# Neos-codes/microbeast

Measured on AMD Instinct MI355X. Metric: env frames/sec (whole node) on 16x16 microRTS, higher is better.
Workload: dtype bf16

## Files before the change

### microbeast_amd/csrc/env/microrts_sim.cpp

```cpp
#include "microrts_sim.h"
#include "../include/microrts_rules.h"
#include <algorithm>
#include <cstring>
#include <cstdlib>
#include <stdexcept>

namespace mb {

#define MB_SPEC(t)                                                                          \
  {(int16_t)mbr::spec_hp(t), (int16_t)mbr::spec_cost(t), (int16_t)mbr::spec_damage(t),      \
   (int16_t)mbr::spec_range(t), (int16_t)mbr::spec_move_t(t), (int16_t)mbr::spec_attack_t(t), \
   (int16_t)mbr::spec_produce_t(t)}
const UnitSpec kSpec[8] = {MB_SPEC(0), MB_SPEC(1), MB_SPEC(2), MB_SPEC(3),
                           MB_SPEC(4), MB_SPEC(5), MB_SPEC(6), MB_SPEC(7)};
#undef MB_SPEC
static constexpr int kHarvestT = mbr::kHarvestT, kReturnT = mbr::kReturnT;
static constexpr int kDX[4] = {0, 1, 0, -1};
static constexpr int kDY[4] = {-1, 0, 1, 0};

enum { R_WIN = 0, R_RES = 1, R_WORKER = 2, R_BUILD = 3, R_ATTACK = 4, R_COMBAT = 5 };

static inline void setbit(uint32_t* w, int j) { w[j >> 5] |= 1u << (j & 31); }
static inline bool getbit(const uint32_t* w, int j) { return (w[j >> 5] >> (j & 31)) & 1u; }

MicroRTSSim::MicroRTSSim(int size, int max_steps, int bot, uint64_t seed, const float* rw)
    : s_(size), max_steps_(max_steps), bot_(bot) {
  if (size < 1 || size > 32) throw std::invalid_argument("MicroRTSSim: map size must be 1..32");
  static const float def[kNumRewards] = {10.f, 1.f, 1.f, 0.2f, 1.f, 4.f};
  for (int i = 0; i < kNumRewards; ++i) rw_[i] = rw ? rw[i] : def[i];
  uint64_t z = seed + 0x9E3779B97F4A7C15ull;
  z = (z ^ (z >> 30)) * 0xBF58476D1CE4E5B9ull;
  z = (z ^ (z >> 27)) * 0x94D049BB133111EBull;
  rng_ = (z ^ (z >> 31)) | 1ull;
  grid_.assign(s_ * s_, -1);
  act_buf_.assign((size_t)s_ * s_ * kActComps, 0);
  mask_.assign(s_ * s_ * kMaskWords, 0u);
  mask_p1_.assign(s_ * s_ * kMaskWords, 0u);
  opp_actions_.assign(s_ * s_ * kActComps, 0);
  reset();
}

uint32_t MicroRTSSim::rand_u32() {
  rng_ ^= rng_ << 13; rng_ ^= rng_ >> 7; rng_ ^= rng_ << 17;
  return (uint32_t)(rng_ >> 16);
}
float MicroRTSSim::rand_unit() { return (rand_u32() & 0xFFFFFF) * (1.f / 16777216.f); }

int MicroRTSSim::add_unit(int type, int owner, int x, int y, int res) {
  Unit u{};
  u.x = x; u.y = y; u.type = type; u.owner = owner;
  u.hp = kSpec[type].hp; u.res = res; u.busy = 0; u.act = A_NOOP; u.alive = 1;
  int uid = -1;
  for (size_t i = 0; i < units_.size(); ++i)
    if (!units_[i].alive) { uid = (int)i; break; }
  if (uid < 0) { uid = (int)units_.size(); units_.push_back(u); }
  else units_[uid] = u;
  grid_[cell(x, y)] = (int16_t)uid;
  if (owner >= 0) ++cnt_[owner][type];
  last_add_ = uid;
  return uid;
}

void MicroRTSSim::kill(int uid) {
  Unit& u = units_[uid];
  if (!u.alive) return;
  grid_[cell(u.x, u.y)] = -1;
  u.alive = 0;
  if (u.owner >= 0) --cnt_[u.owner][u.type];
}

void MicroRTSSim::reset() {
  units_.clear();
  units_.reserve((size_t)s_ * s_ + 4);
  std::memset(cnt_, 0, sizeof(cnt_));
  std::fill(grid_.begin(), grid_.end(), (int16_t)-1);
  tick_ = 0;
  resources_[0] = resources_[1] = 5;
  const int o = s_ >= 8 ? 1 : 0;
  const int b = s_ >= 8 ? 2 : 1;
  for (int p = 0; p < 2; ++p) {
    auto X = [&](int x) { return p == 0 ? x : s_ - 1 - x; };
    auto Y = [&](int y) { return p == 0 ? y : s_ - 1 - y; };
    add_unit(RESOURCE, -1, X(0), Y(0), s_ >= 8 ? 20 : 10);
    if (s_ >= 8) add_unit(RESOURCE, -1, X(0), Y(1), 20);
    add_unit(BASE, p, X(b), Y(b));
    add_unit(WORKER, p, X(o), Y(b == 1 ? 0 : o), 0);
    if (s_ >= 12) add_unit(WORKER, p, X(b + 1), Y(b), 0);
  }
  if (validate_) compute_mask(0, mask_);
  if (external_opp_ && validate_) compute_mask(1, mask_p1_);
}

void MicroRTSSim::unit_mask(const Unit& u, int player, uint32_t* w) const {
  w[0] = w[1] = w[2] = 0;
  if (!u.alive || u.owner != player || u.busy > 0 || u.type == RESOURCE) return;
  const UnitSpec& sp = kSpec[u.type];
  setbit(w, kNvecOff[0] + A_NOOP);
  bool any_move = false, any_harv = false, any_ret = false, any_prod = false, any_att = false;
  const bool mobile = u.type >= WORKER;
  for (int d = 0; d < 4; ++d) {
    int nx = u.x + kDX[d], ny = u.y + kDY[d];
    if (!in_bounds(nx, ny)) continue;
    int g = grid_[cell(nx, ny)];
    if (g < 0) {
      if (mobile) { setbit(w, kNvecOff[1] + d); any_move = true; }
      bool can_prod = false;
      if (u.type == BASE && resources_[player] >= kSpec[WORKER].cost) can_prod = true;
      if (u.type == BARRACKS && resources_[player] >= kSpec[LIGHT].cost) can_prod = true;
      if (u.type == WORKER && resources_[player] >= kSpec[BARRACKS].cost) can_prod = true;
      if (can_prod) { setbit(w, kNvecOff[4] + d); any_prod = true; }
    } else {
      const Unit& t = units_[g];
      if (u.type == WORKER && t.type == RESOURCE && u.res == 0 && t.res > 0) {
        setbit(w, kNvecOff[2] + d); any_harv = true;
      }
      if (u.type == WORKER && t.type == BASE && t.owner == player && u.res > 0) {
        setbit(w, kNvecOff[3] + d); any_ret = true;
      }
    }
  }
  if (any_prod) {
    const int r = resources_[player];
    if (u.type == BASE) setbit(w, kNvecOff[5] + (WORKER - 1));
    if (u.type == BARRACKS) {
      if (r >= kSpec[LIGHT].cost) setbit(w, kNvecOff[5] + (LIGHT - 1));
      if (r >= kSpec[HEAVY].cost) setbit(w, kNvecOff[5] + (HEAVY - 1));
      if (r >= kSpec[RANGED].cost) setbit(w, kNvecOff[5] + (RANGED - 1));
    }
    if (u.type == WORKER) {
      if (r >= kSpec[BASE].cost) setbit(w, kNvecOff[5] + (BASE - 1));
      if (r >= kSpec[BARRACKS].cost) setbit(w, kNvecOff[5] + (BARRACKS - 1));
    }
  }
  if (sp.damage > 0) {
    const int R = sp.range, Rs = std::min(R, 3);
    for (int ay = -Rs; ay <= Rs; ++ay)
      for (int ax = -Rs; ax <= Rs; ++ax) {
        if (ax * ax + ay * ay > R * R || (ax == 0 && ay == 0)) continue;
        int tx = u.x + ax, ty = u.y + ay;
        if (!in_bounds(tx, ty)) continue;
        int g = grid_[cell(tx, ty)];
        if (g >= 0 && units_[g].owner == 1 - player) {
          setbit(w, kNvecOff[6] + (ay + 3) * 7 + (ax + 3)); any_att = true;
        }
      }
  }
  if (any_move) setbit(w, kNvecOff[0] + A_MOVE);
  if (any_harv) setbit(w, kNvecOff[0] + A_HARVEST);
  if (any_ret) setbit(w, kNvecOff[0] + A_RETURN);
  if (any_prod) setbit(w, kNvecOff[0] + A_PRODUCE);
  if (any_att) setbit(w, kNvecOff[0] + A_ATTACK);
}

static void mirror_mask_bits(const uint32_t* in, uint32_t* out) {
  out[0] = out[1] = out[2] = 0;
  for (int j = 0; j < kMaskBits; ++j) {
    if (!getbit(in, j)) continue;
    int k = j;
    if (j >= kNvecOff[1] && j < kNvecOff[5]) {
      int g = (j - kNvecOff[1]) / 4, d = (j - kNvecOff[1]) % 4;
      k = kNvecOff[1] + g * 4 + (d + 2) % 4;
    } else if (j >= kNvecOff[6]) {
      int a = j - kNvecOff[6];
      k = kNvecOff[6] + (6 - a / 7) * 7 + (6 - a % 7);
    }
    setbit(out, k);
  }
}

void MicroRTSSim::map_xy(int player, int x, int y, int* ox, int* oy) const {
  if (player == 0) { *ox = x; *oy = y; }
  else { *ox = s_ - 1 - x; *oy = s_ - 1 - y; }
}

void MicroRTSSim::compute_mask(int player, std::vector<uint32_t>& out) const {
  std::fill(out.begin(), out.end(), 0u);
  for (const Unit& u : units_) {
    if (!u.alive || u.owner != player || u.busy > 0) continue;
    uint32_t w[3];
    unit_mask(u, player, w);
    int px, py;
    map_xy(player, u.x, u.y, &px, &py);
    uint32_t* dst = &out[(size_t)cell(px, py) * kMaskWords];
    if (player == 0) { dst[0] = w[0]; dst[1] = w[1]; dst[2] = w[2]; }
    else mirror_mask_bits(w, dst);
  }
}

bool MicroRTSSim::exec(int uid, const uint8_t* a, float* rw) {
  Unit& u = units_[uid];
  if (!u.alive || u.busy > 0) return false;
  const int player = u.owner;
  const UnitSpec& sp = kSpec[u.type];
  switch (a[0]) {
    case A_NOOP: return true;
    case A_MOVE: {
      if (u.type < WORKER) return false;
      int d = a[1] & 3, nx = u.x + kDX[d], ny = u.y + kDY[d];
      if (!empty(nx, ny)) return false;
      grid_[cell(u.x, u.y)] = -1;
      u.x = nx; u.y = ny;
      grid_[cell(nx, ny)] = (int16_t)uid;
      u.busy = sp.move_t; u.act = A_MOVE;
      return true;
    }
    case A_HARVEST: {
      int d = a[2] & 3, nx = u.x + kDX[d], ny = u.y + kDY[d];
      if (u.type != WORKER || u.res > 0 || !in_bounds(nx, ny)) return false;
      int g = grid_[cell(nx, ny)];
      if (g < 0 || units_[g].type != RESOURCE || units_[g].res <= 0) return false;
      units_[g].res -= 1; u.res = 1;
      if (units_[g].res <= 0) kill(g);
      u.busy = kHarvestT; u.act = A_HARVEST;
      if (rw) rw[R_RES] += 1.f;
      return true;
    }
    case A_RETURN: {
      int d = a[3] & 3, nx = u.x + kDX[d], ny = u.y + kDY[d];
      if (u.type != WORKER || u.res <= 0 || !in_bounds(nx, ny)) return false;
      int g = grid_[cell(nx, ny)];
      if (g < 0 || units_[g].type != BASE || units_[g].owner != player) return false;
      resources_[player] += u.res; u.res = 0;
      u.busy = kReturnT; u.act = A_RETURN;
      if (rw) rw[R_RES] += 1.f;
      return true;
    }
    case A_PRODUCE: {
      int d = a[4] & 3, nx = u.x + kDX[d], ny = u.y + kDY[d];
      int t = (int)a[5] + 1;
      if (t < 1 || t > 7 || !empty(nx, ny)) return false;
      bool ok = (u.type == BASE && t == WORKER) ||
                (u.type == BARRACKS && (t == LIGHT || t == HEAVY || t == RANGED)) ||
                (u.type == WORKER && (t == BASE || t == BARRACKS));
      if (!ok || resources_[player] < kSpec[t].cost) return false;
      resources_[player] -= kSpec[t].cost;
      int nu = add_unit(t, player, nx, ny);
      Unit& uu = units_[uid];
      units_[nu].busy = kSpec[t].produce_t;
      units_[nu].act = A_PRODUCE;
      uu.busy = kSpec[t].produce_t; uu.act = A_PRODUCE;
      if (rw) {
        if (t == WORKER) rw[R_WORKER] += 1.f;
        else if (t == BASE || t == BARRACKS) rw[R_BUILD] += 1.f;
        else rw[R_COMBAT] += 1.f;
      }
      return true;
    }
    case A_ATTACK: {
      if (sp.damage <= 0) return false;
      int ax = (int)(a[6] % 7) - 3, ay = (int)(a[6] / 7) - 3;
      if (ax * ax + ay * ay > sp.range * sp.range) return false;
      int tx = u.x + ax, ty = u.y + ay;
      if (!in_bounds(tx, ty)) return false;
      int g = grid_[cell(tx, ty)];
      if (g < 0 || units_[g].owner != 1 - player) return false;
      units_[g].hp -= sp.damage;
      if (units_[g].hp <= 0) kill(g);
      u.busy = sp.attack_t; u.act = A_ATTACK;
      if (rw) rw[R_ATTACK] += 1.f;
      return true;
    }
  }
  return false;
}

int MicroRTSSim::nearest(int uid, int owner_filter, int type_filter, int* dist) const {
  const Unit& u = units_[uid];
  int best = -1, bd = 1 << 30;
  for (size_t i = 0; i < units_.size(); ++i) {
    const Unit& t = units_[i];
    if (!t.alive || (int)i == uid) continue;
    if (owner_filter != -2 && t.owner != owner_filter) continue;
    if (type_filter > 0 && t.type != type_filter) continue;
    int d = std::abs(t.x - u.x) + std::abs(t.y - u.y);
    if (d < bd) { bd = d; best = (int)i; }
  }
  if (dist) *dist = bd;
  return best;
}

int MicroRTSSim::dir_toward(const Unit& u, int tx, int ty) const {
  int best = -1, bd = 1 << 30;
  const int d0 = std::abs(tx - u.x) + std::abs(ty - u.y);
  for (int d = 0; d < 4; ++d) {
    int nx = u.x + kDX[d], ny = u.y + kDY[d];
    if (!empty(nx, ny)) continue;
    int dd = std::abs(tx - nx) + std::abs(ty - ny);
    if (dd < bd) { bd = dd; best = d; }
  }
  if (best < 0 || bd < d0) return best;
  const int S = s_ * s_;
  int16_t dist[32 * 32];
  int16_t q[32 * 32];
  if (S > 32 * 32) return best;
  std::fill(dist, dist + S, (int16_t)-1);
  int qh = 0, qt = 0;
  const int tc = cell(tx, ty);
  dist[tc] = 0;
  q[qt++] = (int16_t)tc;
  while (qh < qt) {
    const int c = q[qh++], cx = c % s_, cy = c / s_;
    for (int d = 0; d < 4; ++d) {
      const int nx = cx + kDX[d], ny = cy + kDY[d];
      if (!in_bounds(nx, ny)) continue;
      const int nc = cell(nx, ny);
      if (dist[nc] >= 0) continue;
      if (nx == u.x && ny == u.y) {
        for (int k = 0; k < 4; ++k)
          if (u.x + kDX[k] == cx && u.y + kDY[k] == cy) return empty(cx, cy) ? k : best;
      }
      if (grid_[nc] >= 0) continue;
      dist[nc] = (int16_t)(dist[c] + 1);
      q[qt++] = (int16_t)nc;
    }
  }
  return best;
}

static constexpr int kCoacWorkers = 8, kCoacHarvesters = 1;
static constexpr int kLightWorkers = 3;
static constexpr bool kChaseBaseFirst = true;
static constexpr int kChaseBaseSlack = 3;
static constexpr int kRBToward = 8;
static constexpr bool kHuntNoBase = true;
static constexpr bool kHuntAll = false;

void MicroRTSSim::bot_unit(int uid, int player, float* rwo, int n_workers, int n_barracks,
                           int widx) {
  Unit& u = units_[uid];
  uint8_t a[7] = {0, 0, 0, 0, 0, 0, 0};
  const int enemy = 1 - player;
  auto try_attack = [&]() -> bool {
    const UnitSpec& sp = kSpec[u.type];
    if (sp.damage <= 0) return false;
    int best = -1, bkey = 1 << 30;
    const int Rs = std::min<int>(sp.range, 3);
    for (int ay = -Rs; ay <= Rs; ++ay)
      for (int ax = -Rs; ax <= Rs; ++ax) {
        if (ax * ax + ay * ay > sp.range * sp.range || (ax == 0 && ay == 0)) continue;
        int tx = u.x + ax, ty = u.y + ay;
        if (!in_bounds(tx, ty)) continue;
        int g = grid_[cell(tx, ty)];
        if (g >= 0 && units_[g].owner == enemy) {
          const Unit& t = units_[g];
          const int key = (kSpec[t.type].damage > 0 ? 0 : 64) + t.hp;
          if (key < bkey) { bkey = key; best = (ay + 3) * 7 + (ax + 3); }
        }
      }
    if (best < 0) return false;
    a[0] = A_ATTACK; a[6] = (uint8_t)best;
    return exec(uid, a, rwo);
  };
  auto move_to = [&](int tx, int ty) -> bool {
    int d = dir_toward(u, tx, ty);
    if (d < 0) return false;
    a[0] = A_MOVE; a[1] = (uint8_t)d;
    return exec(uid, a, rwo);
  };
  auto produce = [&](int type) -> bool {
    for (int k = 0; k < 4; ++k) {
      int d = (int)((rand_u32() + k) & 3);
      if (!empty(u.x + kDX[d], u.y + kDY[d])) continue;
      a[0] = A_PRODUCE; a[4] = (uint8_t)d; a[5] = (uint8_t)(type - 1);
      return exec(uid, a, rwo);
    }
    return false;
  };
  auto harvest_cycle = [&]() -> bool {
    if (u.res > 0) {
      int dist, b = nearest(uid, player, BASE, &dist);
      if (b < 0) return false;
      if (dist == 1) {
        for (int d = 0; d < 4; ++d)
          if (u.x + kDX[d] == units_[b].x && u.y + kDY[d] == units_[b].y) {
            a[0] = A_RETURN; a[3] = (uint8_t)d; return exec(uid, a, rwo);
          }
      }
      return move_to(units_[b].x, units_[b].y);
    }
    int dist, r = nearest(uid, -1, RESOURCE, &dist);
    if (r < 0) return false;
    if (dist == 1) {
      for (int d = 0; d < 4; ++d)
        if (u.x + kDX[d] == units_[r].x && u.y + kDY[d] == units_[r].y) {
          a[0] = A_HARVEST; a[2] = (uint8_t)d; return exec(uid, a, rwo);
        }
    }
    return move_to(units_[r].x, units_[r].y);
  };
  auto chase = [&]() -> bool {
    int e = -1, dist = 1 << 30, b = -1, db = 1 << 30;
    for (size_t i = 0; i < units_.size(); ++i) {
      const Unit& t = units_[i];
      if (!t.alive || t.owner != enemy) continue;
      const int d = std::abs(t.x - u.x) + std::abs(t.y - u.y);
      if (d < dist) { dist = d; e = (int)i; }
      if (t.type == BASE && d < db) { db = d; b = (int)i; }
    }
    if (e < 0) return false;
    if (kChaseBaseFirst && b >= 0 && db <= dist + kChaseBaseSlack) e = b;
    return move_to(units_[e].x, units_[e].y);
  };

  switch (bot_) {
    case BOT_PASSIVE: return;
    case BOT_RANDOM_BIASED: {
      if (kHuntNoBase && u.type >= WORKER && count_units(enemy, BASE) == 0) {
        if (try_attack()) return;
        if (chase()) return;
      }
      uint32_t w[3];
      unit_mask(u, player, w);
      struct Cand { uint8_t t, p0, p1; };
      Cand cand[4 + 4 + 4 + 4 * 7 + 49 + 1];
      int wt[sizeof(cand) / sizeof(cand[0])], n = 0, tot = 0;
      auto add = [&](uint8_t t, uint8_t p0, uint8_t p1, int weight) {
        cand[n] = {t, p0, p1};
        wt[n++] = weight;
        tot += weight;
      };
      add(A_NOOP, 0, 0, 1);
      int ed = -1, ex = 0, ey = 0;
      if (kRBToward > 1 && u.type >= WORKER) {
        const int e = nearest(uid, 1 - player, -1, &ed);
        if (e >= 0) { ex = units_[e].x; ey = units_[e].y; } else { ed = -1; }
      }
      for (int d = 0; d < 4; ++d) {
        if (getbit(w, kNvecOff[1] + d)) {
          const int nd = std::abs(ex - (u.x + kDX[d])) + std::abs(ey - (u.y + kDY[d]));
          add(A_MOVE, (uint8_t)d, 0, ed >= 0 && nd < ed ? kRBToward : 1);
        }
        if (getbit(w, kNvecOff[2] + d)) add(A_HARVEST, (uint8_t)d, 0, 5);
        if (getbit(w, kNvecOff[3] + d)) add(A_RETURN, (uint8_t)d, 0, 5);
        if (getbit(w, kNvecOff[4] + d))
          for (int k = 0; k < 7; ++k)
            if (getbit(w, kNvecOff[5] + k)) add(A_PRODUCE, (uint8_t)d, (uint8_t)k, 1);
      }
      if (getbit(w, kNvecOff[0] + A_ATTACK))
        for (int j = 0; j < 49; ++j)
          if (getbit(w, kNvecOff[6] + j)) add(A_ATTACK, (uint8_t)j, 0, 5);
      int r = (int)(rand_u32() % (uint32_t)tot), k = 0;
      while (r >= wt[k]) r -= wt[k++];
      const Cand c = cand[k];
      if (c.t == A_NOOP) return;
      a[0] = c.t;
      switch (c.t) {
        case A_MOVE: a[1] = c.p0; break;
        case A_HARVEST: a[2] = c.p0; break;
        case A_RETURN: a[3] = c.p0; break;
        case A_PRODUCE: a[4] = c.p0; a[5] = c.p1; break;
        case A_ATTACK: a[6] = c.p0; break;
        default: break;
      }
      exec(uid, a, rwo);
      return;
    }
    case BOT_RANDOM: {
      uint32_t w[3];
      unit_mask(u, player, w);
      int at = A_NOOP;
      {
        int c[6], n = 0;
        for (int k = 0; k < 6; ++k) if (getbit(w, k)) c[n++] = k;
        at = n ? c[rand_u32() % n] : A_NOOP;
      }
      a[0] = (uint8_t)at;
      int comps[2] = {0, 0}, nc = 0;
      switch (at) {
        case A_MOVE: comps[nc++] = 1; break;
        case A_HARVEST: comps[nc++] = 2; break;
        case A_RETURN: comps[nc++] = 3; break;
        case A_PRODUCE: comps[nc++] = 4; comps[nc++] = 5; break;
        case A_ATTACK: comps[nc++] = 6; break;
        default: break;
      }
      for (int k = 0; k < nc; ++k) {
        const int comp = comps[k];
        int cand[49], n = 0;
        for (int j = 0; j < kNvec[comp]; ++j)
          if (getbit(w, kNvecOff[comp] + j)) cand[n++] = j;
        a[comp] = n ? (uint8_t)cand[rand_u32() % n] : 0;
      }
      if (at != A_NOOP) exec(uid, a, rwo);
      return;
    }
    case BOT_WORKER_RUSH: {
      if (u.type == BASE) { produce(WORKER); return; }
      if (u.type == WORKER) {
        if (try_attack()) return;
        if (widx == 0 && !(kHuntAll && count_units(enemy, BASE) == 0) && harvest_cycle()) return;
        chase();
      }
      return;
    }
    case BOT_LIGHT_RUSH: {
      if (u.type == BASE) { if (n_workers < kLightWorkers) produce(WORKER); return; }
      if (u.type == BARRACKS) { produce(LIGHT); return; }
      if (u.type == WORKER) {
        if (try_attack()) return;
        if (n_barracks == 0 && resources_[player] >= kSpec[BARRACKS].cost && widx == 0) {
          if (produce(BARRACKS)) return;
        }
        if (widx < kLightWorkers - 1 && harvest_cycle()) return;
        chase();
        return;
      }
      if (try_attack()) return;
      chase();
      return;
    }
    case BOT_COAC:
    default: {
      if (u.type == BASE) { if (n_workers < kCoacWorkers) produce(WORKER); return; }
      if (u.type == BARRACKS) {
        const int r = resources_[player];
        int t = (r >= kSpec[HEAVY].cost && rand_unit() < 0.3f) ? HEAVY
              : (rand_unit() < 0.5f ? RANGED : LIGHT);
        produce(t);
        return;
      }
      if (u.type == WORKER) {
        if (try_attack()) return;
        if (n_barracks == 0 && n_workers >= kCoacWorkers / 2 &&
            resources_[player] >= kSpec[BARRACKS].cost && widx == 1) {
          if (produce(BARRACKS)) return;
        }
        if (widx < kCoacHarvesters && !(kHuntAll && count_units(enemy, BASE) == 0) &&
            harvest_cycle())
          return;
        chase();
        return;
      }
      if (try_attack()) return;
      chase();
      return;
    }
  }
}

void MicroRTSSim::bot_act(int player, float* rwo) {
  const int n_workers = cnt_[player][WORKER], n_barracks = cnt_[player][BARRACKS];
  const int n = (int)units_.size();
  uint16_t cand[32 * 32 + 4], cw[32 * 32 + 4], added[32 * 32 + 4];
  int nc = 0, w = 0, na = 0;
  for (int i = 0; i < n; ++i) {
    const Unit& u = units_[i];
    const int own = (u.alive != 0) & (u.owner == player);
    cand[nc] = (uint16_t)i;
    cw[nc] = (uint16_t)w;
    nc += own & (u.busy == 0);
    w += own & (u.type == WORKER);
  }
  for (int q = 0; q < nc; ++q) {
    const int i = cand[q];
    int widx = cw[q];
    for (int t = 0; t < na; ++t) widx += added[t] < i;
    last_add_ = -1;
    bot_unit(i, player, rwo, n_workers, n_barracks, widx);
    const int k = last_add_;
    if (k > i && k < n && units_[k].type == WORKER && units_[k].owner == player)
      added[na++] = (uint16_t)k;
  }
}

void MicroRTSSim::set_opponent_actions(const uint8_t* a) {
  std::memcpy(opp_actions_.data(), a, opp_actions_.size());
}

float MicroRTSSim::step(const uint8_t* actions, bool* done, float* raw) {
  float rw[kNumRewards] = {0, 0, 0, 0, 0, 0};
  const int nc = s_ * s_;
  uint32_t idle[32 * 32 + 4];
  int n_idle = 0;
  for (size_t i = 0; i < units_.size(); ++i) {
    const Unit& u = units_[i];
    idle[n_idle] = ((uint32_t)cell(u.x, u.y) << 16) | (uint32_t)i;
    n_idle += (u.alive != 0) & (u.owner == 0) & (u.busy == 0);
  }
  for (int q = 1; q < n_idle; ++q) {
    const uint32_t key = idle[q];
    int j = q;
    for (; j > 0 && idle[j - 1] > key; --j) idle[j] = idle[j - 1];
    idle[j] = key;
  }
  for (int q = 0; q < n_idle; ++q) {
    const uint32_t key = idle[q];
    const int c = (int)(key >> 16), g = (int)(key & 0xFFFFu);
    uint8_t tmp[kActComps];
    const uint8_t* a = actions + (size_t)c * kActComps;
    if (p16_) {
      mbr::unpack_env_action(p16_[c], tmp);
      a = tmp;
    }
    if (!validate_) {
      if (a[0] < 6) exec(g, a, rw);
      continue;
    }
    const uint32_t* m = &mask_[(size_t)c * kMaskWords];
    if (a[0] >= 6 || !getbit(m, a[0])) continue;
    int comp = 0;
    switch (a[0]) {
      case A_MOVE: comp = 1; break; case A_HARVEST: comp = 2; break;
      case A_RETURN: comp = 3; break; case A_PRODUCE: comp = 4; break;
      case A_ATTACK: comp = 6; break; default: comp = 0;
    }
    if (comp && (a[comp] >= kNvec[comp] || !getbit(m, kNvecOff[comp] + a[comp]))) continue;
    if (a[0] == A_PRODUCE && (a[5] >= 7 || !getbit(m, kNvecOff[5] + a[5]))) continue;
    exec(g, a, rw);
  }
  if (external_opp_) {
    for (int c = 0; c < nc; ++c) {
      int rx, ry;
      map_xy(1, c % s_, c / s_, &rx, &ry);
      const int g = grid_[cell(rx, ry)];
      if (g < 0) continue;
      const Unit& u = units_[g];
      if (u.owner != 1 || u.busy > 0) continue;
      uint8_t otmp[kActComps];
      const uint8_t* ap = &opp_actions_[(size_t)c * kActComps];
      if (opp16_) {
        mbr::unpack_env_action(opp16_[c], otmp);
        ap = otmp;
      }
      if (ap[0] >= 6) continue;
      if (validate_ && !getbit(&mask_p1_[(size_t)c * kMaskWords], ap[0])) continue;
      uint8_t a[7];
      for (int k = 0; k < 7; ++k) a[k] = ap[k];
      for (int k = 1; k <= 4; ++k) a[k] = (uint8_t)((ap[k] + 2) & 3);
      a[6] = (uint8_t)((6 - ap[6] / 7) * 7 + (6 - ap[6] % 7));
      exec(g, a, nullptr);
    }
  } else {
    bot_act(1, nullptr);
  }
  ++tick_;
  int alive[2] = {0, 0};
  for (int t = 0; t < 8; ++t) {
    alive[0] += cnt_[0][t];
    alive[1] += cnt_[1][t];
  }
  bool d = false;
  if (alive[1] == 0 || alive[0] == 0) {
    d = true;
    last_winner_ = alive[1] == 0 ? (alive[0] == 0 ? -1 : 0) : 1;
    rw[R_WIN] = last_winner_ == 0 ? 1.f : (last_winner_ == 1 ? -1.f : 0.f);
  } else if (tick_ >= max_steps_) {
    d = true;
    last_winner_ = -1;
  }
  int rows_n = 0, rows_idle = 0;
  if (!d && rows_out_) {
    uint32_t spill;
    for (Unit& u : units_) {
      const int16_t b = u.busy, nb = (int16_t)(b - (u.alive && b > 0));
      u.act = (b > 0 && nb == 0 && u.alive) ? (int8_t)A_NOOP : u.act;
      u.busy = nb;
      const int live = u.alive != 0;
      rows_idle += live & (u.owner == 0) & (u.act == A_NOOP);
      *(rows_n < nc ? rows_out_ + rows_n : &spill) = row_entry(u, 0);
      rows_n += live;
    }
  } else if (!d) {
    for (Unit& u : units_) {
      const int16_t b = u.busy, nb = (int16_t)(b - (u.alive && b > 0));
      u.act = (b > 0 && nb == 0 && u.alive) ? (int8_t)A_NOOP : u.act;
      u.busy = nb;
    }
  }
  float r = 0.f;
  for (int i = 0; i < kNumRewards; ++i) r += rw_[i] * rw[i];
  if (raw) for (int i = 0; i < kNumRewards; ++i) raw[i] = rw[i];
  *done = d;
  if (d) {
    reset();
    if (rows_out_) rows_n = write_obs_code_list(rows_out_, &rows_idle);
  }
  rows_n_ = rows_n;
  rows_idle_ = rows_idle;
  if (!d) {
    if (validate_) compute_mask(0, mask_);
    if (external_opp_ && validate_) compute_mask(1, mask_p1_);
  }
  return r;
}

float MicroRTSSim::step_packed_list(const uint16_t* env_actions, bool* done, uint32_t* entries,
                                    int* n, int* idle_own) {
  rows_out_ = entries;
  const float r = step_packed(env_actions, done);
  rows_out_ = nullptr;
  *n = rows_n_;
  if (idle_own) *idle_own += rows_idle_;
  return r;
}

float MicroRTSSim::step_packed2_list(const uint16_t* env_actions, const uint16_t* opp_actions,
                                     bool* done, uint32_t* entries, int* n, int* idle_own) {
  rows_out_ = entries;
  const float r = step_packed2(env_actions, opp_actions, done);
  rows_out_ = nullptr;
  *n = rows_n_;
  if (idle_own) *idle_own += rows_idle_;
  return r;
}

float MicroRTSSim::step_packed(const uint16_t* env_actions, bool* done) {
  p16_ = env_actions;
  const float r = step(nullptr, done, nullptr);
  p16_ = nullptr;
  return r;
}

float MicroRTSSim::step_packed2(const uint16_t* env_actions, const uint16_t* opp_actions,
                                bool* done) {
  opp16_ = opp_actions;
  const float r = step_packed(env_actions, done);
  opp16_ = nullptr;
  return r;
}

void MicroRTSSim::write_obs_codes_as(int player, uint16_t* out) const {
  const int nc = s_ * s_;
  std::memset(out, 0, (size_t)nc * sizeof(uint16_t));
  for (const Unit& u : units_) {
    if (!u.alive) continue;
    int px, py;
    map_xy(player, u.x, u.y, &px, &py);
    const int own = u.owner < 0 ? 0 : (u.owner == player ? 1 : 2);
    out[cell(px, py)] = mbr::cell_code(std::min<int>(std::max<int>(u.hp, 0), 4),
                                       std::min<int>(std::max<int>(u.res, 0), 4), own, u.type,
                                       u.act);
  }
}

int MicroRTSSim::write_obs_code_list(uint32_t* entries, int* idle_own, int player) const {
  const int S = s_ * s_;
  uint32_t spill;
  int n = 0, idle = 0;
  for (const Unit& u : units_) {
    const int live = u.alive != 0;
    idle += live & (u.owner == player) & (u.act == A_NOOP);
    *(n < S ? entries + n : &spill) = row_entry(u, player);
    n += live;
  }
  if (idle_own) *idle_own += idle;
  return n;
}

static inline uint32_t unit_bits(const Unit* u, int player) {
  if (!u) return (1u << 0) | (1u << 5) | (1u << 10) | (1u << 13) | (1u << 21);
  uint32_t b = 0;
  b |= 1u << (0 + std::min<int>(std::max<int>(u->hp, 0), 4));
  b |= 1u << (5 + std::min<int>(std::max<int>(u->res, 0), 4));
  int own = u->owner < 0 ? 0 : (u->owner == player ? 1 : 2);
  b |= 1u << (10 + own);
  b |= 1u << (13 + u->type);
  b |= 1u << (21 + u->act);
  return b;
}

void MicroRTSSim::write_obs(uint32_t* out) const {
  const int nc = s_ * s_;
  for (int c = 0; c < nc; ++c) {
    int g = grid_[c];
    out[c] = unit_bits(g >= 0 ? &units_[g] : nullptr, 0);
  }
}

void MicroRTSSim::write_obs_p1(uint32_t* out) const {
  const int nc = s_ * s_;
  for (int c = 0; c < nc; ++c) {
    int rx, ry;
    map_xy(1, c % s_, c / s_, &rx, &ry);
    int g = grid_[cell(rx, ry)];
    out[c] = unit_bits(g >= 0 ? &units_[g] : nullptr, 1);
  }
}

void MicroRTSSim::write_mask(uint32_t* out) const {
  std::memcpy(out, mask_.data(), mask_.size() * sizeof(uint32_t));
}
void MicroRTSSim::write_mask_p1(uint32_t* out) const {
  std::memcpy(out, mask_p1_.data(), mask_p1_.size() * sizeof(uint32_t));
}

void MicroRTSSim::write_obs_dense(float* out) const {
  const int nc = s_ * s_;
  for (int c = 0; c < nc; ++c) {
    int g = grid_[c];
    uint32_t b = unit_bits(g >= 0 ? &units_[g] : nullptr, 0);
    for (int p = 0; p < kPlanes; ++p) out[(size_t)c * kPlanes + p] = (float)((b >> p) & 1u);
  }
}

void MicroRTSSim::write_mask_dense(uint8_t* out) const {
  const int nc = s_ * s_;
  for (int c = 0; c < nc; ++c)
    for (int j = 0; j < kMaskBits; ++j)
      out[(size_t)c * kMaskBits + j] = getbit(&mask_[(size_t)c * kMaskWords], j) ? 1 : 0;
}

}
```

### microbeast_amd/csrc/env/microrts_sim.h

```cpp
#pragma once
#include <cstdint>
#include <vector>
#include <string>

namespace mb {

constexpr int kPlanes = 27;
constexpr int kMaskBits = 78;
constexpr int kMaskWords = 3;
constexpr int kActComps = 7;
constexpr int kNvec[kActComps] = {6, 4, 4, 4, 4, 7, 49};
constexpr int kNvecOff[kActComps + 1] = {0, 6, 10, 14, 18, 22, 29, 78};
constexpr int kNumRewards = 6;

enum UnitType : int8_t { NONE = 0, RESOURCE = 1, BASE = 2, BARRACKS = 3, WORKER = 4,
                         LIGHT = 5, HEAVY = 6, RANGED = 7 };
enum ActType : int8_t { A_NOOP = 0, A_MOVE = 1, A_HARVEST = 2, A_RETURN = 3,
                        A_PRODUCE = 4, A_ATTACK = 5 };
enum Bot : int8_t { BOT_COAC = 0, BOT_RANDOM_BIASED = 1, BOT_LIGHT_RUSH = 2,
                    BOT_WORKER_RUSH = 3, BOT_PASSIVE = 4, BOT_RANDOM = 5 };

struct Unit {
  int16_t x, y;
  int8_t type;
  int8_t owner;
  int16_t hp;
  int16_t res;
  int16_t busy;
  int8_t act;
  int8_t alive;
};

struct SimStats {
  float ep_return = 0.f;
  int32_t ep_step = 0;
};

class MicroRTSSim {
 public:
  MicroRTSSim(int size, int max_steps, int bot, uint64_t seed,
              const float* reward_weight );
  void reset();
  float step(const uint8_t* actions, bool* done, float* raw_rewards );
  void write_obs(uint32_t* out) const;
  void write_mask(uint32_t* out) const;
  void write_obs_dense(float* out) const;
  void write_mask_dense(uint8_t* out) const;
  int size() const { return s_; }
  void prefetch() const {
    const char* u = (const char*)units_.data();
    for (size_t o = 0; o < units_.size() * sizeof(Unit); o += 64) __builtin_prefetch(u + o);
    const char* g = (const char*)grid_.data();
    for (size_t o = 0; o < grid_.size() * sizeof(int16_t); o += 64) __builtin_prefetch(g + o);
  }
  int bot() const { return bot_; }
  void set_bot(int b) { bot_ = b; }
  int winner() const { return last_winner_; }
  int ticks() const { return tick_; }
  void set_external_opponent(bool on) {
    external_opp_ = on;
    if (on && validate_) compute_mask(1, mask_p1_);
  }
  void write_obs_p1(uint32_t* out) const;
  void write_mask_p1(uint32_t* out) const;
  void set_opponent_actions(const uint8_t* actions_p1);
  void set_validate(bool on) {
    validate_ = on;
    if (on) {
      compute_mask(0, mask_);
      if (external_opp_) compute_mask(1, mask_p1_);
    }
  }
  float step_packed(const uint16_t* env_actions, bool* done);
  float step_packed_list(const uint16_t* env_actions, bool* done, uint32_t* entries, int* n,
                         int* idle_own);
  float step_packed2_list(const uint16_t* env_actions, const uint16_t* opp_actions, bool* done,
                          uint32_t* entries, int* n, int* idle_own);
  float step_packed2(const uint16_t* env_actions, const uint16_t* opp_actions, bool* done);
  void write_obs_codes(uint16_t* out) const { write_obs_codes_as(0, out); }
  int write_obs_code_list(uint32_t* entries, int* idle_own = nullptr, int player = 0) const;
  void write_obs_codes_as(int player, uint16_t* out) const;
  bool external_opponent() const { return external_opp_; }
  int resources(int player) const { return resources_[player]; }
  int count_units(int owner, int type) const {
    if (owner < 0 || owner > 1) {
      int n = 0;
      for (const Unit& u : units_) n += u.alive && u.owner == owner && (type < 0 || u.type == type);
      return n;
    }
    if (type >= 0) return cnt_[owner][type];
    int n = 0;
    for (int t = 0; t < 8; ++t) n += cnt_[owner][t];
    return n;
  }

 private:
  int s_, max_steps_, bot_;
  uint64_t rng_;
  float rw_[kNumRewards];
  int tick_ = 0;
  int resources_[2] = {0, 0};
  int last_winner_ = -1;
  bool external_opp_ = false;
  bool validate_ = true;
  std::vector<uint8_t> act_buf_;
  std::vector<Unit> units_;
  std::vector<int16_t> grid_;
  std::vector<uint32_t> mask_;
  std::vector<uint32_t> mask_p1_;
  std::vector<uint8_t> opp_actions_;
  int cnt_[2][8] = {};
  const uint16_t* p16_ = nullptr;
  const uint16_t* opp16_ = nullptr;
  uint32_t* rows_out_ = nullptr;
  int rows_n_ = 0, rows_idle_ = 0;
  int last_add_ = -1;

  uint32_t rand_u32();
  float rand_unit();
  int cell(int x, int y) const { return y * s_ + x; }
  uint32_t row_entry(const Unit& u, int player) const {
    const int px = player ? s_ - 1 - u.x : u.x, py = player ? s_ - 1 - u.y : u.y;
    const int own = u.owner < 0 ? 0 : (u.owner == player ? 1 : 2);
    const int hp = u.hp < 0 ? 0 : (u.hp > 4 ? 4 : u.hp);
    const int res = u.res < 0 ? 0 : (u.res > 4 ? 4 : u.res);
    return (uint32_t)cell(px, py) |
           ((uint32_t)(hp | (res << 3) | (own << 6) | (u.type << 8) | (u.act << 11)) << 16);
  }
  bool in_bounds(int x, int y) const { return x >= 0 && y >= 0 && x < s_ && y < s_; }
  bool empty(int x, int y) const { return in_bounds(x, y) && grid_[cell(x, y)] < 0; }
  int add_unit(int type, int owner, int x, int y, int res = 0);
  void kill(int uid);
  void compute_mask(int player, std::vector<uint32_t>& out) const;
  void unit_mask(const Unit& u, int player, uint32_t* w) const;
  bool exec(int uid, const uint8_t* a, float* rw);
  void bot_act(int player, float* rw_opp);
  void bot_unit(int uid, int player, float* rw_opp, int n_workers, int n_barracks, int widx);
  int nearest(int uid, int owner_filter, int type_filter, int* dist) const;
  int dir_toward(const Unit& u, int tx, int ty) const;
  void map_xy(int player, int x, int y, int* ox, int* oy) const;
};

struct UnitSpec { int16_t hp, cost, damage, range, move_t, attack_t, produce_t; };
extern const UnitSpec kSpec[8];

}
```

### microbeast_amd/csrc/runtime/engine.cpp

```cpp
#include "engine.h"


#include <chrono>
#include <cstdlib>

#include <pthread.h>
#include <sched.h>
#include <cstring>
#include <stdexcept>
#include <string>

#include "../include/mbk_api.h"

namespace mb {

#define ENG_CHECK(expr)                                                              \
  do {                                                                               \
    hipError_t _e = (expr);                                                          \
    if (_e != hipSuccess) {                                                          \
      fail(std::string(#expr) + " failed: " + hipGetErrorString(_e));                \
      return false;                                                                  \
    }                                                                                \
  } while (0)

#define CTOR_CHECK(expr)                                                             \
  do {                                                                               \
    hipError_t _e = (expr);                                                          \
    if (_e != hipSuccess)                                                            \
      throw std::runtime_error(std::string(#expr) + " failed: " + hipGetErrorString(_e)); \
  } while (0)

GpuEngine::GpuEngine(const EngineConfig& cfg, const EngineBuffers& buf) : cfg_(cfg), buf_(buf) {
  if (cfg_.n_groups < 1 || cfg_.envs_per_group < 1 || cfg_.unroll < 1)
    throw std::runtime_error("GpuEngine: bad config");
  if (cfg_.n_slots < cfg_.n_groups + 1)
    throw std::runtime_error("GpuEngine: need n_slots >= n_groups + 1");
  S_ = cfg_.size * cfg_.size;
  const size_t E = cfg_.envs_per_group, T1 = cfg_.unroll + 1;
  slot_stride_obs_ = T1 * E * S_ * 4;
  slot_stride_mask_ = T1 * E * S_ * 4 * kMaskWords;
  slot_stride_act_ = T1 * E * S_ * kActComps;
  slot_stride_scalar_ = T1 * E;
  const int total = cfg_.n_groups * cfg_.envs_per_group;
  env_.reset(new VecEnv(cfg_.size, total, cfg_.max_steps, cfg_.seed, cfg_.bots,
                        cfg_.reward_weight.empty() ? nullptr : cfg_.reward_weight.data(),
                        cfg_.env_index_base));
  CTOR_CHECK(hipSetDevice(cfg_.device));
  if (cfg_.n_lanes < 1 || (int)buf_.lanes.size() != cfg_.n_lanes)
    throw std::runtime_error("GpuEngine: need one LaneIO per lane");
  int prio_least = 0, prio_greatest = 0;
  CTOR_CHECK(hipDeviceGetStreamPriorityRange(&prio_least, &prio_greatest));
  lanes_.resize(cfg_.n_lanes);
  for (int l = 0; l < cfg_.n_lanes; ++l) {
    Lane& L = lanes_[l];
    L.io = buf_.lanes[l];
    if (!L.io.in_codes || !L.io.in_res || !L.io.out_act16)
      throw std::runtime_error("GpuEngine: in_codes / in_res / out_act16 buffers required");
    CTOR_CHECK(hipStreamCreateWithPriority(&L.stream, hipStreamNonBlocking, prio_greatest));
  }
  CTOR_CHECK(hipHostMalloc((void**)&h_codes_, (size_t)total * S_ * 2, hipHostMallocDefault));
  CTOR_CHECK(hipHostMalloc((void**)&h_res_, (size_t)total * 4, hipHostMallocDefault));
  CTOR_CHECK(hipHostMalloc((void**)&h_act16_, (size_t)total * S_ * 2, hipHostMallocDefault));
  CTOR_CHECK(hipHostMalloc((void**)&h_reward_, (size_t)total * 4, hipHostMallocDefault));
  CTOR_CHECK(hipHostMalloc((void**)&h_done_, (size_t)total, hipHostMallocDefault));
  std::memset(h_reward_, 0, (size_t)total * 4);
  std::memset(h_done_, 0, (size_t)total);
  if (buf_.ep_return || buf_.ep_step) {
    CTOR_CHECK(hipHostMalloc((void**)&h_ep_return_, (size_t)total * 4, hipHostMallocDefault));
    CTOR_CHECK(hipHostMalloc((void**)&h_ep_step_, (size_t)total * 4, hipHostMallocDefault));
    std::memset(h_ep_return_, 0, (size_t)total * 4);
    std::memset(h_ep_step_, 0, (size_t)total * 4);
  }
  if (cfg_.selfplay_groups < 0 || cfg_.selfplay_groups > cfg_.n_groups)
    throw std::runtime_error("GpuEngine: bad selfplay_groups");
  const int sp0 = cfg_.n_groups - cfg_.selfplay_groups;
  if (cfg_.selfplay_groups > 0) {
    for (const Lane& L : lanes_)
      if (!L.io.in_codes_p1 || !L.io.in_res_p1 || !L.io.out_act16_p1)
        throw std::runtime_error(
            "GpuEngine: self-play needs in_codes_p1 / in_res_p1 / out_act16_p1");
    CTOR_CHECK(hipHostMalloc((void**)&h_codes_p1_, (size_t)total * S_ * 2, hipHostMallocDefault));
    CTOR_CHECK(hipHostMalloc((void**)&h_res_p1_, (size_t)total * 4, hipHostMallocDefault));
    CTOR_CHECK(hipHostMalloc((void**)&h_act16_p1_, (size_t)total * S_ * 2, hipHostMallocDefault));
    std::memset(h_act16_p1_, 0, (size_t)total * S_ * 2);
    env_->set_external_opponent(sp0 * cfg_.envs_per_group, total, true);
  }
  if (cfg_.preroll > 1) {
    env_->reset_codes(nullptr, nullptr);
    preroll_steps_ = env_->preroll(cfg_.preroll, cfg_.seed, std::max(1, cfg_.n_threads));
    env_->set_validate(false);
    env_->write_codes(h_codes_, h_res_);
  } else {
    env_->set_validate(false);
    env_->reset_codes(h_codes_, h_res_);
  }
  if (cfg_.selfplay_groups > 0) env_->reset_codes_p1(h_codes_p1_, h_res_p1_);
  {
    const char* st = std::getenv("MBK_STEP_TIMING");
    step_timing_ = st && st[0] == '1';
  }
  for (int g = 0; g < cfg_.n_groups; ++g) {
    groups_.emplace_back(new Group());
    CTOR_CHECK(hipEventCreateWithFlags(&groups_[g]->ev, hipEventDisableTiming));
    if (step_timing_)
      for (auto& e : groups_[g]->tev) CTOR_CHECK(hipEventCreate(&e));
    groups_[g]->selfplay = g >= sp0;
    groups_[g]->lane = g % cfg_.n_lanes;
    groups_[g]->phase.store(READY);
  }
  full_ev_.resize(cfg_.n_slots);
  release_ev_.resize(cfg_.n_slots);
  release_pending_.assign(cfg_.n_slots, 0);
  slot_version_.assign(cfg_.n_slots, 0);
  for (int s = 0; s < cfg_.n_slots; ++s) {
    CTOR_CHECK(hipEventCreateWithFlags(&full_ev_[s], hipEventDisableTiming));
    CTOR_CHECK(hipEventCreateWithFlags(&release_ev_[s], hipEventDisableTiming));
    free_slots_.push_back(s);
  }
  for (PubChan& c : pub_) {
    CTOR_CHECK(hipEventCreateWithFlags(&c.ready, hipEventDisableTiming));
    c.pending.assign(cfg_.n_lanes, false);
    c.dst.assign(cfg_.n_lanes, 0);
    c.consumed.assign(cfg_.n_lanes, nullptr);
    for (auto& ev : c.consumed) CTOR_CHECK(hipEventCreateWithFlags(&ev, hipEventDisableTiming));
  }
  chunk_ = std::max(1, std::min(16, cfg_.envs_per_group / std::max(1, 2 * cfg_.n_threads)));
}

GpuEngine::~GpuEngine() {
  stop();
  for (Lane& L : lanes_)
    if (L.stream) hipStreamSynchronize(L.stream);
  for (auto& g : groups_) {
    if (g->ev) hipEventDestroy(g->ev);
    for (auto e : g->tev)
      if (e) hipEventDestroy(e);
  }
  for (auto e : full_ev_) hipEventDestroy(e);
  for (auto e : release_ev_) hipEventDestroy(e);
  for (PubChan& c : pub_) {
    if (c.ready) hipEventDestroy(c.ready);
    for (auto ev : c.consumed)
      if (ev) hipEventDestroy(ev);
    if (c.staging) hipFree(c.staging);
  }
  if (h_codes_p1_) hipHostFree(h_codes_p1_);
  if (h_res_p1_) hipHostFree(h_res_p1_);
  if (h_act16_p1_) hipHostFree(h_act16_p1_);
  if (h_codes_) hipHostFree(h_codes_);
  if (h_res_) hipHostFree(h_res_);
  if (h_act16_) hipHostFree(h_act16_);
  if (h_reward_) hipHostFree(h_reward_);
  if (h_ep_return_) hipHostFree(h_ep_return_);
  if (h_ep_step_) hipHostFree(h_ep_step_);
  if (h_done_) hipHostFree(h_done_);
  if (h_code_list_) hipHostFree(h_code_list_);
  if (h_act_list_) hipHostFree(h_act_list_);
  if (h_code_list_p1_) hipHostFree(h_code_list_p1_);
  if (h_act_list_p1_) hipHostFree(h_act_list_p1_);
  for (Lane& L : lanes_) {
    if (L.opp_scratch) hipFree(L.opp_scratch);
    if (L.stream) hipStreamDestroy(L.stream);
  }
}

void GpuEngine::fail(const std::string& msg) {
  {
    std::lock_guard<std::mutex> g(err_m_);
    if (err_.empty()) err_ = msg;
  }
  failed_.store(true);
  running_.store(false);
  work_cv_.notify_all();
  full_cv_.notify_all();
}

std::string GpuEngine::error() const {
  std::lock_guard<std::mutex> g(err_m_);
  return err_;
}

void GpuEngine::start(const std::vector<LaneGraphs>& graphs) {
  if (running_.load()) return;
  if ((int)graphs.size() != cfg_.n_lanes)
    throw std::runtime_error("GpuEngine::start: need one LaneGraphs per lane");
  for (int l = 0; l < cfg_.n_lanes; ++l) {
    const LaneGraphs& g = graphs[l];
    if (!g.policy) throw std::runtime_error("GpuEngine::start: missing policy graph");
    if (cfg_.selfplay_groups > 0 && !g.opp)
      throw std::runtime_error("GpuEngine::start: self-play groups need the opponent graph");
    Lane& L = lanes_[l];
    L.graph = (hipGraphExec_t)g.policy;
    L.opp_graph = (hipGraphExec_t)g.opp;
    L.pack_graph[0] = (hipGraphExec_t)g.pack;
    L.pack_graph[1] = (hipGraphExec_t)g.opp_pack;
  }
  started_ = true;
  running_.store(true);
  for (int w = 0; w < cfg_.n_threads; ++w) workers_.emplace_back(&GpuEngine::worker_loop, this, w);
  driver_ = std::thread(&GpuEngine::driver_loop, this);
}

void GpuEngine::alloc_rows() {
  if (h_code_list_) return;
  const size_t total = (size_t)cfg_.n_groups * cfg_.envs_per_group;
  list_stride_ = (S_ + 1 + 3) & ~3;
  const size_t bytes = total * list_stride_ * 4;
  if (hipHostMalloc((void**)&h_code_list_, bytes, hipHostMallocDefault) != hipSuccess ||
      hipHostMalloc((void**)&h_act_list_, bytes, hipHostMallocDefault) != hipSuccess)
    throw std::runtime_error("GpuEngine: hipHostMalloc of the sparse rows failed");
  std::memset(h_act_list_, 0, bytes);
  env_->write_code_lists(h_code_list_, list_stride_);
  if (cfg_.selfplay_groups > 0) {
    if (hipHostMalloc((void**)&h_code_list_p1_, bytes, hipHostMallocDefault) != hipSuccess ||
        hipHostMalloc((void**)&h_act_list_p1_, bytes, hipHostMallocDefault) != hipSuccess)
      throw std::runtime_error("GpuEngine: hipHostMalloc of the opponent rows failed");
    std::memset(h_act_list_p1_, 0, bytes);
    std::memset(h_code_list_p1_, 0, bytes);
    env_->write_code_lists(h_code_list_p1_, list_stride_, 1);
  }
}

void GpuEngine::set_greedy(bool on) {
  if (started_ || running_.load()) throw std::runtime_error("set_greedy: engine already started");
  greedy_ = on;
}

void GpuEngine::set_sparse_io(bool on) {
  if (running_.load()) throw std::runtime_error("set_sparse_io: engine running");
  if (!on) { sparse_ = false; return; }
  if (act_mode()) return;
  if (buf_.ep_return || buf_.ep_step)
    throw std::runtime_error("set_sparse_io: not with the reference buffer keys");
  alloc_rows();
  sparse_ = true;
}

void GpuEngine::set_act_models(const std::vector<MbkActModel>& models,
                               const std::vector<MbkActModel>& opp_models) {
  if (running_.load()) throw std::runtime_error("set_act_models: engine running");
  if (!models.empty() && (int)models.size() != cfg_.n_lanes)
    throw std::runtime_error("set_act_models: need one model per lane");
  if (!models.empty() && (buf_.ep_return || buf_.ep_step || buf_.last_action0 || buf_.logits))
    throw std::runtime_error("set_act_models: not with reference buffer keys");
  const bool sp_needed = !models.empty() && cfg_.selfplay_groups > 0;
  if (sp_needed && (int)opp_models.size() != cfg_.n_lanes)
    throw std::runtime_error("set_act_models: self-play needs one opponent block per lane");
  if (!sp_needed && !opp_models.empty())
    throw std::runtime_error("set_act_models: opponent blocks without self-play groups");
  for (const std::vector<MbkActModel>* v : {&models, &opp_models})
    for (const MbkActModel& m : *v)
      if (m.E != cfg_.envs_per_group || m.H != cfg_.size || m.W != cfg_.size)
        throw std::runtime_error("set_act_models: model block shape mismatch");
  act_models_ = models;
  opp_act_models_ = opp_models;
  sparse_ = !models.empty();
  if (sparse_) alloc_rows();
  if (sp_needed) {
    const size_t E = cfg_.envs_per_group, sc = E * S_ * (4 + 12 + 8) + 2 * E * 4 + 256;
    for (Lane& L : lanes_)
      if (!L.opp_scratch && hipMalloc((void**)&L.opp_scratch, sc) != hipSuccess)
        throw std::runtime_error("set_act_models: hipMalloc of the opponent scratch failed");
  }
}

void GpuEngine::stop() {
  running_.store(false);
  work_cv_.notify_all();
  full_cv_.notify_all();
  if (driver_.joinable()) driver_.join();
  for (auto& t : workers_) if (t.joinable()) t.join();
  workers_.clear();
  for (Lane& L : lanes_)
    if (L.stream) hipStreamSynchronize(L.stream);
}

void GpuEngine::dispatch_env(int g) {
  Group& G = *groups_[g];
  const auto now = std::chrono::steady_clock::now();
  gpu_phase_ns_.fetch_add(
      std::chrono::duration_cast<std::chrono::nanoseconds>(now - G.t_phase).count(),
      std::memory_order_relaxed);
  G.t_phase = now;
  if (G.timed) {
    float ms[3] = {0.f, 0.f, 0.f};
    bool ok = true;
    for (int i = 0; i < 3; ++i)
      ok = ok && hipEventElapsedTime(&ms[i], G.tev[i], G.tev[i + 1]) == hipSuccess;
    if (ok) {
      step_h2d_ns_.fetch_add((int64_t)(ms[0] * 1e6), std::memory_order_relaxed);
      step_graph_ns_.fetch_add((int64_t)(ms[1] * 1e6), std::memory_order_relaxed);
      step_out_ns_.fetch_add((int64_t)(ms[2] * 1e6), std::memory_order_relaxed);
      timed_steps_.fetch_add(1, std::memory_order_relaxed);
    }
    G.timed = false;
  }
  G.idle.store(0, std::memory_order_relaxed);
  G.phase.store(ENV_BUSY, std::memory_order_release);
  G.remaining.store(cfg_.envs_per_group, std::memory_order_release);
  G.next_env.store(0, std::memory_order_release);
  {
    std::lock_guard<std::mutex> l(work_m_);
    work_epoch_.fetch_add(1);
  }
  work_cv_.notify_all();
}

void GpuEngine::worker_loop(int wid) {
  const int E = cfg_.envs_per_group, NG = cfg_.n_groups;
  while (running_.load(std::memory_order_relaxed)) {
    const uint64_t epoch = work_epoch_.load();
    bool did = false;
    for (int k = 0; k < NG; ++k) {
      const int g = (wid + k) % NG;
      Group& G = *groups_[g];
      if (G.phase.load(std::memory_order_acquire) != ENV_BUSY) continue;
      for (;;) {
        int e = G.next_env.fetch_add(chunk_);
        if (e >= E) break;
        int e1 = std::min(e + chunk_, E);
        const int a0 = g * E;
        auto t0 = std::chrono::steady_clock::now();
        try {
          if (inject_fault_.exchange(0) != 0)
            throw std::runtime_error("injected env-worker fault (--fault_inject_every)");
          if (sparse_ && G.selfplay)
            G.idle.fetch_add(env_->step_range_lists_sp(a0 + e, a0 + e1, h_act_list_,
                                                       h_act_list_p1_, h_code_list_,
                                                       h_code_list_p1_, list_stride_, h_reward_,
                                                       h_done_, &log_, G.opp_version),
                             std::memory_order_relaxed);
          else if (sparse_)
            G.idle.fetch_add(env_->step_range_lists(a0 + e, a0 + e1, h_act_list_, h_code_list_,
                                                    list_stride_, h_reward_, h_done_, &log_),
                             std::memory_order_relaxed);
          else if (G.selfplay)
            env_->step_range_codes_sp(a0 + e, a0 + e1, h_act16_, h_act16_p1_, h_codes_, h_res_,
                                      h_codes_p1_, h_res_p1_, h_reward_, h_done_, &log_,
                                      G.opp_version, h_ep_return_, h_ep_step_);
          else
            env_->step_range_codes(a0 + e, a0 + e1, h_act16_, h_codes_, h_res_, h_reward_,
                                   h_done_, &log_, h_ep_return_, h_ep_step_);
        } catch (const std::exception& ex) {
          fail("env worker " + std::to_string(wid) + ": " + ex.what());
          return;
        }
        env_ns_.fetch_add(std::chrono::duration_cast<std::chrono::nanoseconds>(
                              std::chrono::steady_clock::now() - t0).count(),
                          std::memory_order_relaxed);
        frames_.fetch_add(e1 - e, std::memory_order_relaxed);
        did = true;
        if (G.remaining.fetch_sub(e1 - e) == e1 - e) {
          G.t_ready_ns.store(std::chrono::duration_cast<std::chrono::nanoseconds>(
                                 std::chrono::steady_clock::now().time_since_epoch()).count(),
                             std::memory_order_relaxed);
          G.phase.store(READY, std::memory_order_release);
        }
      }
    }
    if (!did) {
      std::unique_lock<std::mutex> l(work_m_);
      work_cv_.wait_for(l, std::chrono::milliseconds(2),
                        [&] { return work_epoch_.load() != epoch || !running_.load(); });
    }
  }
}

bool GpuEngine::enqueue_gpu(int g) {
  const auto t_enq = std::chrono::steady_clock::now();
  struct Timer {
    std::atomic<int64_t>& acc;
    std::chrono::steady_clock::time_point t0;
    ~Timer() {
      acc.fetch_add(std::chrono::duration_cast<std::chrono::nanoseconds>(
                        std::chrono::steady_clock::now() - t0).count(),
                    std::memory_order_relaxed);
    }
  } timer{enqueue_ns_, t_enq};
  Group& G = *groups_[g];
  Lane& L = lanes_[G.lane];
  hipStream_t st = L.stream;
  const LaneIO& io = L.io;
  const size_t E = cfg_.envs_per_group, T = cfg_.unroll;
  {
    std::lock_guard<std::mutex> l(pub_m_);
    const int ln = G.lane;
    for (int c = 0; c < 2; ++c) {
      PubChan& P = pub_[c];
      if (!P.pending[ln]) continue;
      if (hipEventQuery(P.ready) == hipErrorNotReady) continue;
      ENG_CHECK(hipStreamWaitEvent(st, P.ready, 0));
      ENG_CHECK(hipMemcpyAsync((void*)P.dst[ln], P.staging, P.n, hipMemcpyDeviceToDevice,
                               st));
      ENG_CHECK(hipEventRecord(P.consumed[ln], st));
      if (L.pack_graph[c]) ENG_CHECK(hipGraphLaunch(L.pack_graph[c], st));
      P.pending[ln] = false;
      if (c == 1) L.opp_version = P.version;
      else if (P.version >= 0) L.policy_version = P.version;
      bool all = true;
      for (bool pl : P.pending) all = all && !pl;
      if (all) {
        if (c == 0) publishes_.fetch_add(1);
        else {
          opp_version_pub_.store(P.version);
          opp_publishes_.fetch_add(1);
        }
      }
    }
  }
  if (G.t == 0) {
    auto waiting = [&] {
      for (int w : slot_wait_q_) if (w == g) return true;
      return false;
    };
    if (!slot_wait_q_.empty() && slot_wait_q_.front() != g) {
      if (!waiting()) slot_wait_q_.push_back(g);
      return false;
    }
    int slot = -1;
    bool pending = false;
    {
      std::lock_guard<std::mutex> l(slot_m_);
      for (auto it = free_slots_.begin(); it != free_slots_.end(); ++it) {
        const int s = *it;
        if (release_pending_[s]) {
          const hipError_t q = hipEventQuery(release_ev_[s]);
          if (q == hipErrorNotReady) continue;
          if (q == hipSuccess) release_pending_[s] = 0;
        }
        slot = s;
        pending = release_pending_[s] != 0;
        free_slots_.erase(it);
        break;
      }
    }
    if (slot < 0) {
      if (!waiting()) slot_wait_q_.push_back(g);
      return false;
    }
    if (!slot_wait_q_.empty() && slot_wait_q_.front() == g) slot_wait_q_.pop_front();
    if (pending) ENG_CHECK(hipStreamWaitEvent(st, release_ev_[slot], 0));
    G.cur = slot;
    slot_version_[slot] = L.policy_version;
  }
  const size_t e0 = (size_t)g * E;
  G.timed = step_timing_;
  const size_t t = G.t;
  auto obs_at = [&](int slot, size_t i) {
    return (char*)buf_.obs + slot * slot_stride_obs_ + i * E * S_ * 4;
  };
  auto mask_at = [&](int slot, size_t i) {
    return (char*)buf_.mask + slot * slot_stride_mask_ + i * E * S_ * 4 * kMaskWords;
  };
  auto act_at = [&](int slot, size_t i) {
    return (char*)buf_.action + slot * slot_stride_act_ + i * E * S_ * kActComps;
  };
  auto f32_at = [&](uintptr_t base, int slot, size_t i) {
    return (char*)base + (slot * slot_stride_scalar_ + i * E) * 4;
  };
  auto u8_at = [&](uintptr_t base, int slot, size_t i) {
    return (char*)base + (slot * slot_stride_scalar_ + i * E);
  };
  const bool close_prev = (t == 0 && G.prev >= 0);
  const int rs = t > 0 ? G.cur : G.prev;
  const size_t ri = t > 0 ? t - 1 : T - 1;
  if (act_mode()) {
    const MbkActModel& M = act_models_[G.lane];
    if (G.timed) ENG_CHECK(hipEventRecord(G.tev[0], st));
    if (G.timed) ENG_CHECK(hipEventRecord(G.tev[1], st));
    MbkActStep a{};
    a.code_list = h_code_list_ + e0 * list_stride_;
    a.act_list = h_act_list_ + e0 * list_stride_;
    a.list_stride = list_stride_;
    a.obs = (uint32_t*)obs_at(G.cur, t);
    a.mask = (uint32_t*)mask_at(G.cur, t);
    if (close_prev) {
      a.obs2 = (uint32_t*)obs_at(G.prev, T);
      a.mask2 = (uint32_t*)mask_at(G.prev, T);
    }
    a.action = (uint8_t*)act_at(G.cur, t);
    if (buf_.abits) {
      const size_t sw = (size_t)(S_ + 31) / 32;
      auto ab_at = [&](int slot, size_t i) {
        return (uint32_t*)buf_.abits + (slot * slot_stride_scalar_ + i * E) * sw;
      };
      a.abits = ab_at(G.cur, t);
      if (close_prev) a.abits2 = ab_at(G.prev, T);
    }
    a.logp = (float*)f32_at(buf_.logp, G.cur, t);
    a.value = (float*)f32_at(buf_.value, G.cur, t);
    if (!G.first) {
      a.reward_src = h_reward_ + e0;
      a.done_src = h_done_ + e0;
      a.reward_dst = (float*)f32_at(buf_.reward, rs, ri);
      a.done_dst = (uint8_t*)u8_at(buf_.done, rs, ri);
    }
    a.step = L.act_step++;
    a.greedy = greedy_ ? 1 : 0;
    act_active_cells_.fetch_add(G.idle.load(std::memory_order_relaxed), std::memory_order_relaxed);
    act_steps_.fetch_add(1, std::memory_order_relaxed);
    {
      const auto t0 = std::chrono::steady_clock::now();
      ENG_CHECK((hipError_t)mbk_act_step(&M, &a, st));
      if (G.selfplay) {
        const size_t ES = E * S_;
        uint8_t* sc = L.opp_scratch;
        MbkActStep o{};
        o.code_list = h_code_list_p1_ + e0 * list_stride_;
        o.act_list = h_act_list_p1_ + e0 * list_stride_;
        o.list_stride = list_stride_;
        o.obs = (uint32_t*)sc;
        o.mask = (uint32_t*)(sc + ES * 4);
        o.action = sc + ES * 16;
        o.logp = (float*)(sc + ES * 24);
        o.value = (float*)(sc + ES * 24 + E * 4);
        o.step = L.opp_act_step++;
        ENG_CHECK((hipError_t)mbk_act_step(&opp_act_models_[G.lane], &o, st));
        G.opp_version = L.opp_version;
      }
      launch_ns_.fetch_add(std::chrono::duration_cast<std::chrono::nanoseconds>(
                               std::chrono::steady_clock::now() - t0).count(),
                           std::memory_order_relaxed);
    }
    if (G.timed) ENG_CHECK(hipEventRecord(G.tev[2], st));
    if (close_prev) {
      ENG_CHECK(hipEventRecord(full_ev_[G.prev], st));
      {
        std::lock_guard<std::mutex> l(slot_m_);
        full_slots_.push_back(G.prev);
      }
      slots_full_.fetch_add(1);
      full_cv_.notify_all();
      G.prev = -1;
    }
    if (G.timed) ENG_CHECK(hipEventRecord(G.tev[3], st));
    ENG_CHECK(hipEventRecord(G.ev, st));
  } else {
    const uintptr_t in_codes = io.in_codes, in_res = io.in_res, out_act16 = io.out_act16;
    if (G.timed) ENG_CHECK(hipEventRecord(G.tev[0], st));
    if (sparse_) {
      ENG_CHECK((hipError_t)mbk_rows_to_codes(h_code_list_ + e0 * list_stride_, list_stride_,
                                              (int)E, S_, (void*)in_codes, (int32_t*)in_res,
                                              st));
    } else {
      ENG_CHECK(hipMemcpyAsync((void*)in_codes, h_codes_ + e0 * S_, E * S_ * 2,
                               hipMemcpyHostToDevice, st));
      ENG_CHECK(hipMemcpyAsync((void*)in_res, h_res_ + e0, E * 4, hipMemcpyHostToDevice, st));
    }
    if (G.timed) ENG_CHECK(hipEventRecord(G.tev[1], st));
    {
      const auto t0 = std::chrono::steady_clock::now();
      ENG_CHECK(hipGraphLaunch(L.graph, st));
      launch_ns_.fetch_add(std::chrono::duration_cast<std::chrono::nanoseconds>(
                               std::chrono::steady_clock::now() - t0).count(),
                           std::memory_order_relaxed);
    }
    if (G.selfplay) {
      if (sparse_) {
        ENG_CHECK((hipError_t)mbk_rows_to_codes(h_code_list_p1_ + e0 * list_stride_,
                                                list_stride_, (int)E, S_, (void*)io.in_codes_p1,
                                                (int32_t*)io.in_res_p1, st));
      } else {
        ENG_CHECK(hipMemcpyAsync((void*)io.in_codes_p1, h_codes_p1_ + e0 * S_, E * S_ * 2,
                                 hipMemcpyHostToDevice, st));
        ENG_CHECK(hipMemcpyAsync((void*)io.in_res_p1, h_res_p1_ + e0, E * 4,
                                 hipMemcpyHostToDevice, st));
      }
      ENG_CHECK(hipGraphLaunch(L.opp_graph, st));
      G.opp_version = L.opp_version;
    }

    if (G.timed) ENG_CHECK(hipEventRecord(G.tev[2], st));
    MbkCopySeg seg[MBK_MAX_COPY_SEGS];
    int n = 0;
    seg[n++] = {(const void*)io.in_obs, obs_at(G.cur, t), E * S_ * 4};
    seg[n++] = {(const void*)io.in_mask, mask_at(G.cur, t), E * S_ * 4 * kMaskWords};
    seg[n++] = {(const void*)io.out_action, act_at(G.cur, t), E * S_ * kActComps};
    seg[n++] = {(const void*)io.out_logp, f32_at(buf_.logp, G.cur, t), E * 4};
    seg[n++] = {(const void*)io.out_value, f32_at(buf_.value, G.cur, t), E * 4};
    if (!G.first) {
      seg[n++] = {(const void*)(h_reward_ + e0), f32_at(buf_.reward, rs, ri), E * 4};
      seg[n++] = {(const void*)(h_done_ + e0), u8_at(buf_.done, rs, ri), E};
      if (buf_.ep_return)
        seg[n++] = {(const void*)(h_ep_return_ + e0), f32_at(buf_.ep_return, rs, ri), E * 4};
      if (buf_.ep_step)
        seg[n++] = {(const void*)(h_ep_step_ + e0), f32_at(buf_.ep_step, rs, ri), E * 4};
    }
    if (buf_.logits && io.out_logits)
      seg[n++] = {(const void*)io.out_logits,
                  (char*)buf_.logits + (G.cur * slot_stride_scalar_ + t * E) * (size_t)S_ * 78 * 4,
                  E * (size_t)S_ * 78 * 4};
    if (close_prev && buf_.last_action0)
      seg[n++] = {(const void*)act_at(G.prev, T - 1),
                  (char*)buf_.last_action0 + (size_t)G.cur * E * S_ * kActComps,
                  E * S_ * kActComps};
    if (close_prev) {
      seg[n++] = {(const void*)io.in_obs, obs_at(G.prev, T), E * S_ * 4};
      seg[n++] = {(const void*)io.in_mask, mask_at(G.prev, T), E * S_ * 4 * kMaskWords};
    }
    ENG_CHECK((hipError_t)mbk_multi_copy(seg, n, st));
    if (close_prev) {
      ENG_CHECK(hipEventRecord(full_ev_[G.prev], st));
      {
        std::lock_guard<std::mutex> l(slot_m_);
        full_slots_.push_back(G.prev);
      }
      slots_full_.fetch_add(1);
      full_cv_.notify_all();
      G.prev = -1;
    }
    if (sparse_) {
      ENG_CHECK((hipError_t)mbk_codes_to_rows((const void*)out_act16, (int)E, S_,
                                              h_act_list_ + e0 * list_stride_, list_stride_,
                                              st));
      if (G.selfplay)
        ENG_CHECK((hipError_t)mbk_codes_to_rows((const void*)io.out_act16_p1, (int)E, S_,
                                                h_act_list_p1_ + e0 * list_stride_,
                                                list_stride_, st));
    } else {
      ENG_CHECK(hipMemcpyAsync(h_act16_ + e0 * S_, (const void*)out_act16, E * S_ * 2,
                               hipMemcpyDeviceToHost, st));
      if (G.selfplay)
        ENG_CHECK(hipMemcpyAsync(h_act16_p1_ + e0 * S_, (const void*)io.out_act16_p1,
                                 E * S_ * 2, hipMemcpyDeviceToHost, st));
    }
    if (G.timed) ENG_CHECK(hipEventRecord(G.tev[3], st));
    ENG_CHECK(hipEventRecord(G.ev, st));
  }
  gpu_steps_.fetch_add(1);
  G.t += 1;
  if (G.t == (int)T) {
    G.t = 0;
    G.prev = G.cur;
    G.cur = -1;
  }
  G.first = false;
  {
    const auto now = std::chrono::steady_clock::now();
    const int64_t rdy = G.t_ready_ns.exchange(0, std::memory_order_relaxed);
    if (rdy > 0)
      env_phase_ns_.fetch_add(
          rdy - std::chrono::duration_cast<std::chrono::nanoseconds>(
                    G.t_phase.time_since_epoch()).count(),
          std::memory_order_relaxed);
    G.t_phase = now;
  }
  G.phase.store(ON_GPU, std::memory_order_release);
  return true;
}

void GpuEngine::driver_loop() {
  hipSetDevice(cfg_.device);
  const int NG = cfg_.n_groups;
  int idle_spins = 0;
  auto idle_t0 = std::chrono::steady_clock::now();
  bool idle = false;
  double stall_s = 0.0;
  while (running_.load(std::memory_order_relaxed)) {
    bool progressed = false, stalled = false;
    for (int g = 0; g < NG && running_.load(std::memory_order_relaxed); ++g) {
      Group& G = *groups_[g];
      int ph = G.phase.load(std::memory_order_acquire);
      if (ph == READY) {
        if (enqueue_gpu(g)) progressed = true;
        else if (failed_.load()) return;
        else stalled = true;
      } else if (ph == ON_GPU) {
        hipError_t q = hipEventQuery(G.ev);
        if (q == hipSuccess) {
          dispatch_env(g);
          progressed = true;
        } else if (q != hipErrorNotReady) {
          fail(std::string("hipEventQuery: ") + hipGetErrorString(q));
          return;
        }
      }
    }
    if (progressed) {
      if (idle) {
        double dt = std::chrono::duration<double>(std::chrono::steady_clock::now() - idle_t0).count();
        std::lock_guard<std::mutex> l(stats_m_);
        driver_idle_s_ += dt;
        if (stall_s > 0) slot_wait_s_ += dt;
      }
      idle = false;
      idle_spins = 0;
      stall_s = 0.0;
    } else {
      if (!idle) { idle = true; idle_t0 = std::chrono::steady_clock::now(); }
      if (stalled) stall_s = 1.0;
      if (++idle_spins < 256) {
        __builtin_ia32_pause();
      } else if (idle_spins < 2048) {
        std::this_thread::yield();
      } else {
        std::this_thread::sleep_for(std::chrono::microseconds(20));
      }
    }
  }
}

std::vector<int> GpuEngine::get_full(int n, double timeout_s) {
  std::unique_lock<std::mutex> l(slot_m_);
  auto pred = [&] { return (int)full_slots_.size() >= n || !running_.load() || failed_.load(); };
  if (timeout_s < 0) full_cv_.wait(l, pred);
  else full_cv_.wait_for(l, std::chrono::duration<double>(timeout_s), pred);
  std::vector<int> out;
  if ((int)full_slots_.size() < n) return out;
  for (int i = 0; i < n; ++i) { out.push_back(full_slots_.front()); full_slots_.pop_front(); }
  return out;
}

void GpuEngine::stream_wait_full(uintptr_t stream, int slot) {
  hipError_t e = hipStreamWaitEvent((hipStream_t)stream, full_ev_[slot], 0);
  if (e != hipSuccess) throw std::runtime_error(std::string("stream_wait_full: ") + hipGetErrorString(e));
}

void GpuEngine::release(const std::vector<int>& slots, uintptr_t stream) {
  for (int s : slots) {
    hipError_t e = hipEventRecord(release_ev_[s], (hipStream_t)stream);
    if (e != hipSuccess) throw std::runtime_error(std::string("release: ") + hipGetErrorString(e));
  }
  std::lock_guard<std::mutex> l(slot_m_);
  for (int s : slots) {
    release_pending_[s] = 1;
    free_slots_.push_back(s);
  }
}

bool GpuEngine::publish_chan(int chan, uintptr_t src, const std::vector<uintptr_t>& dsts,
                             size_t nbytes, uintptr_t stream, int version) {
  std::lock_guard<std::mutex> l(pub_m_);
  PubChan& P = pub_[chan];
  if ((int)dsts.size() != cfg_.n_lanes)
    throw std::runtime_error("publish: need one destination per lane");
  for (bool pl : P.pending)
    if (pl) return false;
  hipStream_t s = (hipStream_t)stream;
  if (nbytes > P.staging_n) {
    if (P.staging) {
      for (Lane& L : lanes_) hipStreamSynchronize(L.stream);
      hipFree(P.staging);
    }
    if (hipMalloc((void**)&P.staging, nbytes) != hipSuccess)
      throw std::runtime_error("publish: hipMalloc staging failed");
    P.staging_n = nbytes;
  }
  for (hipEvent_t ev : P.consumed) hipStreamWaitEvent(s, ev, 0);
  hipMemcpyAsync(P.staging, (const void*)src, nbytes, hipMemcpyDeviceToDevice, s);
  hipEventRecord(P.ready, s);
  P.dst = dsts;
  P.n = nbytes;
  P.version = version;
  P.pending.assign(cfg_.n_lanes, true);
  return true;
}

EngineStats GpuEngine::stats() const {
  EngineStats s;
  s.frames = frames_.load();
  s.gpu_steps = gpu_steps_.load();
  s.slots_full = slots_full_.load();
  s.env_s = env_ns_.load() * 1e-9;
  s.gpu_phase_s = gpu_phase_ns_.load() * 1e-9;
  s.step_h2d_s = step_h2d_ns_.load() * 1e-9;
  s.step_graph_s = step_graph_ns_.load() * 1e-9;
  s.step_out_s = step_out_ns_.load() * 1e-9;
  s.timed_steps = timed_steps_.load();
  s.preroll_steps = preroll_steps_;
  s.env_phase_s = env_phase_ns_.load() * 1e-9;
  s.enqueue_s = enqueue_ns_.load() * 1e-9;
  s.graph_launch_s = launch_ns_.load() * 1e-9;
  s.publishes = publishes_.load();
  s.opp_publishes = opp_publishes_.load();
  s.opp_version = opp_version_pub_.load();
  s.act_steps = act_steps_.load();
  s.act_active_cells = act_active_cells_.load();
  {
    std::lock_guard<std::mutex> q(slot_m_);
    s.full_depth = (int)full_slots_.size();
  }
  std::lock_guard<std::mutex> l(stats_m_);
  s.driver_idle_s = driver_idle_s_;
  s.slot_wait_s = slot_wait_s_;
  return s;
}

}
```

### microbeast_amd/csrc/runtime/vec_env.cpp

```cpp
#include "vec_env.h"

#include <algorithm>
#include <atomic>
#include <random>
#include <thread>

namespace mb {

VecEnv::VecEnv(int size, int n_envs, int max_steps, uint64_t seed, const std::vector<int>& bots,
               const float* rw, int env_index_base)
    : size_(size), base_(env_index_base) {
  for (int i = 0; i < n_envs; ++i) {
    int bot = bots.empty() ? (int)BOT_COAC : bots[i % bots.size()];
    sims_.emplace_back(new MicroRTSSim(size, max_steps, bot,
                                       seed * 1000003ull + (uint64_t)(env_index_base + i), rw));
  }
  ep_ret_.assign(n_envs, 0.f);
  ep_len_.assign(n_envs, 0);
}

void VecEnv::reset(uint32_t* obs, uint32_t* mask) {
  const size_t S = (size_t)size_ * size_;
  for (size_t i = 0; i < sims_.size(); ++i) {
    sims_[i]->reset();
    ep_ret_[i] = 0.f;
    ep_len_[i] = 0;
    if (obs) sims_[i]->write_obs(obs + i * S);
    if (mask) sims_[i]->write_mask(mask + i * S * kMaskWords);
  }
}

void VecEnv::step_range(int e0, int e1, int base, const uint8_t* actions, uint32_t* obs,
                        uint32_t* mask, float* reward, uint8_t* done, float* ep_return,
                        int32_t* ep_step, EpisodeLog* log) {
  const size_t S = (size_t)size_ * size_;
  for (int i = e0; i < e1; ++i) {
    const size_t j = (size_t)(i - base);
    bool d = false;
    float r = sims_[i]->step(actions + j * S * kActComps, &d, nullptr);
    ep_ret_[i] += r;
    ep_len_[i] += 1;
    if (ep_return) ep_return[j] = ep_ret_[i];
    if (ep_step) ep_step[j] = ep_len_[i];
    if (d) {
      if (log) log->push({ep_ret_[i], ep_len_[i], base_ + i, sims_[i]->winner(), -1 - sims_[i]->bot()});
      ep_ret_[i] = 0.f;
      ep_len_[i] = 0;
    }
    if (reward) reward[j] = r;
    if (done) done[j] = d ? 1 : 0;
    if (obs) sims_[i]->write_obs(obs + j * S);
    if (mask) sims_[i]->write_mask(mask + j * S * kMaskWords);
  }
}

void VecEnv::set_validate(bool on) {
  for (auto& s : sims_) s->set_validate(on);
}

void VecEnv::reset_codes(uint16_t* codes, int32_t* res) {
  const size_t S = (size_t)size_ * size_;
  for (size_t i = 0; i < sims_.size(); ++i) {
    sims_[i]->reset();
    ep_ret_[i] = 0.f;
    ep_len_[i] = 0;
    if (codes) sims_[i]->write_obs_codes(codes + i * S);
    if (res) res[i] = sims_[i]->resources(0);
  }
}

void VecEnv::write_codes(uint16_t* codes, int32_t* res) const {
  const size_t S = (size_t)size_ * size_;
  for (size_t i = 0; i < sims_.size(); ++i) {
    sims_[i]->write_obs_codes(codes + i * S);
    res[i] = sims_[i]->resources(0);
  }
}

namespace {
void uniform_legal(const uint32_t* mask, int S, std::mt19937_64& rng, uint8_t* act) {
  for (int c = 0; c < S; ++c) {
    const uint32_t* m = mask + (size_t)c * kMaskWords;
    uint8_t* a = act + (size_t)c * kActComps;
    if ((m[0] | m[1] | m[2]) == 0) {
      for (int k = 0; k < kActComps; ++k) a[k] = 0;
      continue;
    }
    for (int k = 0; k < kActComps; ++k) {
      int cand[49], n = 0;
      for (int j = 0; j < kNvec[k]; ++j) {
        const int b = kNvecOff[k] + j;
        if ((m[b >> 5] >> (b & 31)) & 1u) cand[n++] = j;
      }
      a[k] = n ? (uint8_t)cand[rng() % (uint64_t)n] : 0;
    }
  }
}
}

int64_t VecEnv::preroll(int max_pre, uint64_t seed, int n_threads) {
  if (max_pre <= 1 || sims_.empty()) return 0;
  const int n = (int)sims_.size(), S = size_ * size_;
  std::atomic<int> next{0};
  std::atomic<int64_t> played{0};
  auto work = [&]() {
    std::vector<uint32_t> m(S * kMaskWords), m1(S * kMaskWords);
    std::vector<uint8_t> a(S * kActComps), a1(S * kActComps);
    for (int i; (i = next.fetch_add(1)) < n;) {
      std::mt19937_64 rng(seed * 0x9E3779B97F4A7C15ull + (uint64_t)(base_ + i));
      const int r = (int)(rng() % (uint64_t)max_pre);
      MicroRTSSim& sim = *sims_[i];
      for (int t = 0; t < r; ++t) {
        sim.write_mask(m.data());
        uniform_legal(m.data(), S, rng, a.data());
        if (sim.external_opponent()) {
          sim.write_mask_p1(m1.data());
          uniform_legal(m1.data(), S, rng, a1.data());
          sim.set_opponent_actions(a1.data());
        }
        bool d = false;
        sim.step(a.data(), &d, nullptr);
      }
      ep_ret_[i] = 0.f;
      ep_len_[i] = 0;
      played.fetch_add(r);
    }
  };
  const int nt = std::max(1, std::min(n_threads, n));
  std::vector<std::thread> th;
  for (int k = 1; k < nt; ++k) th.emplace_back(work);
  work();
  for (auto& t : th) t.join();
  return played.load();
}

void VecEnv::reset_codes_p1(uint16_t* codes_p1, int32_t* res_p1) const {
  const size_t S = (size_t)size_ * size_;
  for (size_t i = 0; i < sims_.size(); ++i) {
    if (!sims_[i]->external_opponent()) continue;
    sims_[i]->write_obs_codes_as(1, codes_p1 + i * S);
    res_p1[i] = sims_[i]->resources(1);
  }
}

void VecEnv::step_range_codes(int e0, int e1, const uint16_t* actions, uint16_t* codes,
                              int32_t* res, float* reward, uint8_t* done, EpisodeLog* log,
                              float* ep_return, int32_t* ep_step) {
  const size_t S = (size_t)size_ * size_;
  for (int i = e0; i < e1; ++i) {
    if (i + 2 < e1) __builtin_prefetch(sims_[i + 2].get());
    if (i + 1 < e1) {
      sims_[i + 1]->prefetch();
      for (size_t o = 0; o < S * 2; o += 64) {
        __builtin_prefetch((const char*)(actions + (i + 1) * S) + o);
        __builtin_prefetch((char*)(codes + (i + 1) * S) + o, 1);
      }
    }
    bool d = false;
    const float r = sims_[i]->step_packed(actions + (size_t)i * S, &d);
    ep_ret_[i] += r;
    ep_len_[i] += 1;
    if (ep_return) ep_return[i] = ep_ret_[i];
    if (ep_step) ep_step[i] = ep_len_[i];
    if (d) {
      if (log) log->push({ep_ret_[i], ep_len_[i], base_ + i, sims_[i]->winner(), -1 - sims_[i]->bot()});
      ep_ret_[i] = 0.f;
      ep_len_[i] = 0;
    }
    reward[i] = r;
    done[i] = d ? 1 : 0;
    sims_[i]->write_obs_codes(codes + (size_t)i * S);
    res[i] = sims_[i]->resources(0);
  }
}

void VecEnv::write_code_lists(uint32_t* lists, int stride, int player) const {
  for (size_t i = 0; i < sims_.size(); ++i) {
    if (player != 0 && !sims_[i]->external_opponent()) continue;
    uint32_t* row = lists + i * (size_t)stride;
    const int n = sims_[i]->write_obs_code_list(row + 1, nullptr, player);
    row[0] = (uint32_t)n | ((uint32_t)sims_[i]->resources(player) << 16);
  }
}

int VecEnv::step_range_lists_sp(int e0, int e1, const uint32_t* act_lists,
                                const uint32_t* opp_lists, uint32_t* code_lists,
                                uint32_t* code_lists_p1, int stride, float* reward, uint8_t* done,
                                EpisodeLog* log, int opponent) {
  const size_t S = (size_t)size_ * size_;
  thread_local std::vector<uint16_t> dense, dense_opp;
  dense.assign(S, 0);
  dense_opp.assign(S, 0);
  auto expand = [&](const uint32_t* row, std::vector<uint16_t>& out, uint16_t keep) {
    const uint32_t na = std::min<uint32_t>(row[0] & 0xFFFFu, (uint32_t)S);
    for (uint32_t k = 1; k <= na; ++k) {
      const uint32_t c = row[k] & 0xFFFFu;
      if (c < S) out[c] = keep ? (uint16_t)(row[k] >> 16) : 0;
    }
  };
  int idle = 0;
  for (int i = e0; i < e1; ++i) {
    if (i + 1 < e1) sims_[i + 1]->prefetch();
    MicroRTSSim& sim = *sims_[i];
    const bool sp = sim.external_opponent();
    const uint32_t* arow = act_lists + (size_t)i * stride;
    const uint32_t* orow = opp_lists + (size_t)i * stride;
    expand(arow, dense, 1);
    if (sp) expand(orow, dense_opp, 1);
    bool d = false;
    uint32_t* crow = code_lists + (size_t)i * stride;
    int n = 0;
    const float r = sp ? sim.step_packed2_list(dense.data(), dense_opp.data(), &d, crow + 1, &n, &idle)
                       : sim.step_packed_list(dense.data(), &d, crow + 1, &n, &idle);
    expand(arow, dense, 0);
    if (sp) expand(orow, dense_opp, 0);
    ep_ret_[i] += r;
    ep_len_[i] += 1;
    if (d) {
      if (log) log->push({ep_ret_[i], ep_len_[i], base_ + i, sim.winner(),
                          sp ? opponent : -1 - sim.bot()});
      ep_ret_[i] = 0.f;
      ep_len_[i] = 0;
    }
    reward[i] = r;
    done[i] = d ? 1 : 0;
    crow[0] = (uint32_t)n | ((uint32_t)sim.resources(0) << 16);
    if (sp) {
      uint32_t* prow = code_lists_p1 + (size_t)i * stride;
      const int n1 = sim.write_obs_code_list(prow + 1, nullptr, 1);
      prow[0] = (uint32_t)n1 | ((uint32_t)sim.resources(1) << 16);
    }
  }
  return idle;
}

int VecEnv::step_range_lists(int e0, int e1, const uint32_t* act_lists, uint32_t* code_lists,
                             int stride, float* reward, uint8_t* done, EpisodeLog* log) {
  const size_t S = (size_t)size_ * size_;
  int idle = 0;
  thread_local std::vector<uint16_t> dense;
  dense.assign(S, 0);
  for (int i = e0; i < e1; ++i) {
    if (i + 2 < e1) __builtin_prefetch(sims_[i + 2].get());
    if (i + 1 < e1) {
      sims_[i + 1]->prefetch();
      __builtin_prefetch(act_lists + (size_t)(i + 1) * stride);
    }
    const uint32_t* arow = act_lists + (size_t)i * stride;
    const uint32_t na = std::min<uint32_t>(arow[0] & 0xFFFFu, (uint32_t)S);
    for (uint32_t k = 1; k <= na; ++k) {
      const uint32_t c = arow[k] & 0xFFFFu;
      if (c < S) dense[c] = (uint16_t)(arow[k] >> 16);
    }
    bool d = false;
    uint32_t* crow = code_lists + (size_t)i * stride;
    int n = 0;
    const float r = sims_[i]->step_packed_list(dense.data(), &d, crow + 1, &n, &idle);
    for (uint32_t k = 1; k <= na; ++k) {
      const uint32_t c = arow[k] & 0xFFFFu;
      if (c < S) dense[c] = 0;
    }
    ep_ret_[i] += r;
    ep_len_[i] += 1;
    if (d) {
      if (log) log->push({ep_ret_[i], ep_len_[i], base_ + i, sims_[i]->winner(), -1 - sims_[i]->bot()});
      ep_ret_[i] = 0.f;
      ep_len_[i] = 0;
    }
    reward[i] = r;
    done[i] = d ? 1 : 0;
    crow[0] = (uint32_t)n | ((uint32_t)sims_[i]->resources(0) << 16);
  }
  return idle;
}

void VecEnv::step_range_codes_sp(int e0, int e1, const uint16_t* actions,
                                 const uint16_t* opp_actions, uint16_t* codes, int32_t* res,
                                 uint16_t* codes_p1, int32_t* res_p1, float* reward,
                                 uint8_t* done, EpisodeLog* log, int opponent,
                                 float* ep_return, int32_t* ep_step) {
  const size_t S = (size_t)size_ * size_;
  for (int i = e0; i < e1; ++i) {
    if (i + 2 < e1) __builtin_prefetch(sims_[i + 2].get());
    if (i + 1 < e1) sims_[i + 1]->prefetch();
    MicroRTSSim& sim = *sims_[i];
    const bool sp = sim.external_opponent();
    bool d = false;
    const float r = sp ? sim.step_packed2(actions + (size_t)i * S, opp_actions + (size_t)i * S, &d)
                       : sim.step_packed(actions + (size_t)i * S, &d);
    ep_ret_[i] += r;
    ep_len_[i] += 1;
    if (ep_return) ep_return[i] = ep_ret_[i];
    if (ep_step) ep_step[i] = ep_len_[i];
    if (d) {
      if (log) log->push({ep_ret_[i], ep_len_[i], base_ + i, sim.winner(), sp ? opponent : -1 - sim.bot()});
      ep_ret_[i] = 0.f;
      ep_len_[i] = 0;
    }
    reward[i] = r;
    done[i] = d ? 1 : 0;
    sim.write_obs_codes(codes + (size_t)i * S);
    res[i] = sim.resources(0);
    if (sp) {
      sim.write_obs_codes_as(1, codes_p1 + (size_t)i * S);
      res_p1[i] = sim.resources(1);
    }
  }
}

void VecEnv::set_external_opponent(int e0, int e1, bool on) {
  for (int i = e0; i < e1; ++i) sims_[i]->set_external_opponent(on);
}

void VecEnv::dense_obs(float* out) const {
  const size_t S = (size_t)size_ * size_;
  for (size_t i = 0; i < sims_.size(); ++i) sims_[i]->write_obs_dense(out + i * S * kPlanes);
}

void VecEnv::dense_mask(uint8_t* out) const {
  const size_t S = (size_t)size_ * size_;
  for (size_t i = 0; i < sims_.size(); ++i) sims_[i]->write_mask_dense(out + i * S * kMaskBits);
}

}
```

### microbeast_amd/csrc/runtime/vec_env.h

```cpp
#pragma once
#include <cstdint>
#include <memory>
#include <mutex>
#include <vector>
#include "../env/microrts_sim.h"

namespace mb {

struct EpisodeRecord {
  float ep_return;
  int32_t ep_step;
  int32_t env_index;
  int32_t winner;
  int32_t opponent;
};

class EpisodeLog {
 public:
  void push(const EpisodeRecord& r) {
    std::lock_guard<std::mutex> g(m_);
    recs_.push_back(r);
    ++total_;
  }
  std::vector<EpisodeRecord> drain() {
    std::lock_guard<std::mutex> g(m_);
    std::vector<EpisodeRecord> out;
    out.swap(recs_);
    return out;
  }
  int64_t total() const { return total_; }

 private:
  std::mutex m_;
  std::vector<EpisodeRecord> recs_;
  int64_t total_ = 0;
};

class VecEnv {
 public:
  VecEnv(int size, int n_envs, int max_steps, uint64_t seed, const std::vector<int>& bots,
         const float* reward_weight, int env_index_base = 0);
  int num_envs() const { return (int)sims_.size(); }
  int size() const { return size_; }
  void reset(uint32_t* obs, uint32_t* mask);
  void step_range(int e0, int e1, int base, const uint8_t* actions, uint32_t* obs,
                  uint32_t* mask, float* reward, uint8_t* done, float* ep_return,
                  int32_t* ep_step, EpisodeLog* log);
  void set_validate(bool on);
  void reset_codes(uint16_t* codes, int32_t* res);
  void reset_codes_p1(uint16_t* codes_p1, int32_t* res_p1) const;
  void step_range_codes(int e0, int e1, const uint16_t* actions, uint16_t* codes, int32_t* res,
                        float* reward, uint8_t* done, EpisodeLog* log,
                        float* ep_return = nullptr, int32_t* ep_step = nullptr);
  void write_code_lists(uint32_t* lists, int stride, int player = 0) const;
  int step_range_lists(int e0, int e1, const uint32_t* act_lists, uint32_t* code_lists,
                       int stride, float* reward, uint8_t* done, EpisodeLog* log);
  int step_range_lists_sp(int e0, int e1, const uint32_t* act_lists, const uint32_t* opp_lists,
                          uint32_t* code_lists, uint32_t* code_lists_p1, int stride,
                          float* reward, uint8_t* done, EpisodeLog* log, int opponent);
  void step_range_codes_sp(int e0, int e1, const uint16_t* actions, const uint16_t* opp_actions,
                           uint16_t* codes, int32_t* res, uint16_t* codes_p1, int32_t* res_p1,
                           float* reward, uint8_t* done, EpisodeLog* log, int opponent,
                           float* ep_return = nullptr, int32_t* ep_step = nullptr);
  void set_external_opponent(int e0, int e1, bool on);
  int64_t preroll(int max_pre, uint64_t seed, int n_threads);
  void write_codes(uint16_t* codes, int32_t* res) const;
  void dense_obs(float* out) const;
  void dense_mask(uint8_t* out) const;
  MicroRTSSim& sim(int i) { return *sims_[i]; }
  const std::vector<float>& ep_return() const { return ep_ret_; }
  const std::vector<int32_t>& ep_step() const { return ep_len_; }

 private:
  int size_;
  int base_;
  std::vector<std::unique_ptr<MicroRTSSim>> sims_;
  std::vector<float> ep_ret_;
  std::vector<int32_t> ep_len_;
};

}
```

Measured before the change: 21.56 million.

## Track units with liveness bitsets, arena-allocate sims, and compute masks lazily

Replaces the per-sim unit vector with a fixed arena-backed array. Per-word live, idle and worker bitsets let scans visit only relevant units instead of every slot. Action masks are recomputed lazily on demand rather than after every step, the BFS scratch uses a stamp array instead of refilling, and all sims are placed contiguously in one aligned arena with object-level prefetching. The env worker also batches its atomic counter updates per chunk loop, which adds complexity and risks stale-mask or bitset-consistency bugs.

```diff
diff --git a/microbeast_amd/csrc/env/microrts_sim.cpp b/microbeast_amd/csrc/env/microrts_sim.cpp
--- a/microbeast_amd/csrc/env/microrts_sim.cpp
+++ b/microbeast_amd/csrc/env/microrts_sim.cpp
@@ -4,6 +4,7 @@
 #include <cstring>
 #include <cstdlib>
 #include <stdexcept>
+#include <type_traits>
 
 namespace mb {
 
@@ -23,20 +24,26 @@
 static inline void setbit(uint32_t* w, int j) { w[j >> 5] |= 1u << (j & 31); }
 static inline bool getbit(const uint32_t* w, int j) { return (w[j >> 5] >> (j & 31)) & 1u; }
 
-MicroRTSSim::MicroRTSSim(int size, int max_steps, int bot, uint64_t seed, const float* rw)
+MicroRTSSim::~MicroRTSSim() { std::free(own_state_); }
+
+MicroRTSSim::MicroRTSSim(int size, int max_steps, int bot, uint64_t seed, const float* rw,
+                         void* state)
     : s_(size), max_steps_(max_steps), bot_(bot) {
   if (size < 1 || size > 32) throw std::invalid_argument("MicroRTSSim: map size must be 1..32");
+  if ((size_t)((const char*)&slots_[1] - (const char*)this) > kHotBytes)
+    throw std::logic_error("MicroRTSSim: prefetch_object() no longer covers the step's fields");
   static const float def[kNumRewards] = {10.f, 1.f, 1.f, 0.2f, 1.f, 4.f};
   for (int i = 0; i < kNumRewards; ++i) rw_[i] = rw ? rw[i] : def[i];
   uint64_t z = seed + 0x9E3779B97F4A7C15ull;
   z = (z ^ (z >> 30)) * 0xBF58476D1CE4E5B9ull;
   z = (z ^ (z >> 27)) * 0x94D049BB133111EBull;
   rng_ = (z ^ (z >> 31)) | 1ull;
-  grid_.assign(s_ * s_, -1);
-  act_buf_.assign((size_t)s_ * s_ * kActComps, 0);
-  mask_.assign(s_ * s_ * kMaskWords, 0u);
-  mask_p1_.assign(s_ * s_ * kMaskWords, 0u);
-  opp_actions_.assign(s_ * s_ * kActComps, 0);
+  if (!state) {
+    own_state_ = state = std::aligned_alloc(64, state_bytes(s_));
+    if (!state) throw std::bad_alloc();
+  }
+  grid_ = (int16_t*)state;
+  units_ = (Unit*)((char*)state + grid_bytes(s_));
   reset();
 }
 
@@ -50,11 +57,20 @@
   Unit u{};
   u.x = x; u.y = y; u.type = type; u.owner = owner;
   u.hp = kSpec[type].hp; u.res = res; u.busy = 0; u.act = A_NOOP; u.alive = 1;
-  int uid = -1;
-  for (size_t i = 0; i < units_.size(); ++i)
-    if (!units_[i].alive) { uid = (int)i; break; }
-  if (uid < 0) { uid = (int)units_.size(); units_.push_back(u); }
-  else units_[uid] = u;
+  int uid = n_units_;
+  const int nw = (n_units_ + 63) >> 6;
+  for (int w = 0; w < nw; ++w) {
+    const uint64_t dead = ~(slots_[w].live[0] | slots_[w].live[1] | slots_[w].live[2]);
+    if (dead) {
+      uid = std::min(n_units_, (w << 6) + __builtin_ctzll(dead));
+      break;
+    }
+  }
+  if (uid == n_units_) ++n_units_;
+  units_[uid] = u;
+  SlotWord& sw = slots_[uid >> 6];
+  sw.live[owner + 1] |= 1ull << (uid & 63);
+  if (type == WORKER) sw.worker[owner] |= 1ull << (uid & 63);
   grid_[cell(x, y)] = (int16_t)uid;
   if (owner >= 0) ++cnt_[owner][type];
   last_add_ = uid;
@@ -66,14 +82,22 @@
   if (!u.alive) return;
   grid_[cell(u.x, u.y)] = -1;
   u.alive = 0;
+  SlotWord& sw = slots_[uid >> 6];
+  sw.live[u.owner + 1] &= ~(1ull << (uid & 63));
+  if (u.owner >= 0) {
+    sw.idle[u.owner] &= ~(1ull << (uid & 63));
+    sw.worker[u.owner] &= ~(1ull << (uid & 63));
+  }
   if (u.owner >= 0) --cnt_[u.owner][u.type];
 }
 
 void MicroRTSSim::reset() {
-  units_.clear();
-  units_.reserve((size_t)s_ * s_ + 4);
+  n_units_ = 0;
+  std::memset(slots_, 0, sizeof(slots_));
   std::memset(cnt_, 0, sizeof(cnt_));
-  std::fill(grid_.begin(), grid_.end(), (int16_t)-1);
+  std::fill(grid_, grid_ + s_ * s_, (int16_t)-1);
+  const unsigned nl = (unsigned)(grid_bytes(s_) / 64);
+  grid_lines_ = nl >= 32 ? ~0u : (1u << nl) - 1;
   tick_ = 0;
   resources_[0] = resources_[1] = 5;
   const int o = s_ >= 8 ? 1 : 0;
@@ -87,8 +111,9 @@
     add_unit(WORKER, p, X(o), Y(b == 1 ? 0 : o), 0);
     if (s_ >= 12) add_unit(WORKER, p, X(b + 1), Y(b), 0);
   }
-  if (validate_) compute_mask(0, mask_);
-  if (external_opp_ && validate_) compute_mask(1, mask_p1_);
+  for (int w = 0; w < (n_units_ + 63) >> 6; ++w)
+    for (int p = 0; p < 2; ++p) slots_[w].idle[p] = slots_[w].live[p + 1];
+  mask_stale_ = true;
 }
 
 void MicroRTSSim::unit_mask(const Unit& u, int player, uint32_t* w) const {
@@ -175,8 +200,9 @@
 
 void MicroRTSSim::compute_mask(int player, std::vector<uint32_t>& out) const {
   std::fill(out.begin(), out.end(), 0u);
-  for (const Unit& u : units_) {
-    if (!u.alive || u.owner != player || u.busy > 0) continue;
+  for_owner(player, [&](int i) {
+    const Unit& u = units_[i];
+    if (u.busy > 0) return;
     uint32_t w[3];
     unit_mask(u, player, w);
     int px, py;
@@ -184,7 +210,18 @@
     uint32_t* dst = &out[(size_t)cell(px, py) * kMaskWords];
     if (player == 0) { dst[0] = w[0]; dst[1] = w[1]; dst[2] = w[2]; }
     else mirror_mask_bits(w, dst);
-  }
+  });
+}
+
+void MicroRTSSim::ensure_masks() const {
+  if (mask_.empty()) {
+    mask_.assign((size_t)s_ * s_ * kMaskWords, 0u);
+    mask_p1_.assign((size_t)s_ * s_ * kMaskWords, 0u);
+  }
+  if (!mask_stale_ || !validate_) return;
+  compute_mask(0, mask_);
+  if (external_opp_) compute_mask(1, mask_p1_);
+  mask_stale_ = false;
 }
 
 bool MicroRTSSim::exec(int uid, const uint8_t* a, float* rw) {
@@ -264,17 +301,16 @@
   return false;
 }
 
-int MicroRTSSim::nearest(int uid, int owner_filter, int type_filter, int* dist) const {
+int MicroRTSSim::nearest(int uid, int owner, int type_filter, int* dist) const {
   const Unit& u = units_[uid];
   int best = -1, bd = 1 << 30;
-  for (size_t i = 0; i < units_.size(); ++i) {
-    const Unit& t = units_[i];
-    if (!t.alive || (int)i == uid) continue;
-    if (owner_filter != -2 && t.owner != owner_filter) continue;
-    if (type_filter > 0 && t.type != type_filter) continue;
-    int d = std::abs(t.x - u.x) + std::abs(t.y - u.y);
-    if (d < bd) { bd = d; best = (int)i; }
-  }
+  if (!(owner >= 0 && type_filter > 0 && cnt_[owner][type_filter] == 0))
+    for_owner(owner, [&](int i) {
+      const Unit& t = units_[i];
+      if (i == uid || (type_filter > 0 && t.type != type_filter)) return;
+      const int d = std::abs(t.x - u.x) + std::abs(t.y - u.y);
+      if (d < bd) { bd = d; best = i; }
+    });
   if (dist) *dist = bd;
   return best;
 }
@@ -289,14 +325,19 @@
     if (dd < bd) { bd = dd; best = d; }
   }
   if (best < 0 || bd < d0) return best;
-  const int S = s_ * s_;
-  int16_t dist[32 * 32];
-  int16_t q[32 * 32];
-  if (S > 32 * 32) return best;
-  std::fill(dist, dist + S, (int16_t)-1);
+  struct Scratch { uint16_t seen[32 * 32]; int16_t q[32 * 32]; uint16_t stamp; };
+  thread_local Scratch bfs = {};
+  if (s_ * s_ > 32 * 32) return best;
+  if (++bfs.stamp == 0) {
+    std::memset(bfs.seen, 0, sizeof(bfs.seen));
+    bfs.stamp = 1;
+  }
+  uint16_t* const seen = bfs.seen;
+  int16_t* const q = bfs.q;
+  const uint16_t stamp = bfs.stamp;
   int qh = 0, qt = 0;
   const int tc = cell(tx, ty);
-  dist[tc] = 0;
+  seen[tc] = stamp;
   q[qt++] = (int16_t)tc;
   while (qh < qt) {
     const int c = q[qh++], cx = c % s_, cy = c / s_;
@@ -304,13 +345,13 @@
       const int nx = cx + kDX[d], ny = cy + kDY[d];
       if (!in_bounds(nx, ny)) continue;
       const int nc = cell(nx, ny);
-      if (dist[nc] >= 0) continue;
+      if (seen[nc] == stamp) continue;
       if (nx == u.x && ny == u.y) {
         for (int k = 0; k < 4; ++k)
           if (u.x + kDX[k] == cx && u.y + kDY[k] == cy) return empty(cx, cy) ? k : best;
       }
       if (grid_[nc] >= 0) continue;
-      dist[nc] = (int16_t)(dist[c] + 1);
+      seen[nc] = stamp;
       q[qt++] = (int16_t)nc;
     }
   }
@@ -335,18 +376,32 @@
     if (sp.damage <= 0) return false;
     int best = -1, bkey = 1 << 30;
     const int Rs = std::min<int>(sp.range, 3);
-    for (int ay = -Rs; ay <= Rs; ++ay)
-      for (int ax = -Rs; ax <= Rs; ++ax) {
-        if (ax * ax + ay * ay > sp.range * sp.range || (ax == 0 && ay == 0)) continue;
-        int tx = u.x + ax, ty = u.y + ay;
-        if (!in_bounds(tx, ty)) continue;
-        int g = grid_[cell(tx, ty)];
-        if (g >= 0 && units_[g].owner == enemy) {
-          const Unit& t = units_[g];
-          const int key = (kSpec[t.type].damage > 0 ? 0 : 64) + t.hp;
-          if (key < bkey) { bkey = key; best = (ay + 3) * 7 + (ax + 3); }
+    int n_enemy = 0;
+    for (int t = 0; t < 8; ++t) n_enemy += cnt_[enemy][t];
+    if (Rs > 1 && n_enemy < 12) {
+      int bpair = 1 << 30;
+      for_owner(enemy, [&](int i) {
+        const Unit& t = units_[i];
+        const int ax = t.x - u.x, ay = t.y - u.y;
+        if (ax < -Rs || ax > Rs || ay < -Rs || ay > Rs || ax * ax + ay * ay > sp.range * sp.range)
+          return;
+        const int key = (kSpec[t.type].damage > 0 ? 0 : 64) + t.hp, idx = (ay + 3) * 7 + (ax + 3);
+        if (key * 64 + idx < bpair) { bpair = key * 64 + idx; best = idx; }
+      });
+    } else {
+      for (int ay = -Rs; ay <= Rs; ++ay)
+        for (int ax = -Rs; ax <= Rs; ++ax) {
+          if (ax * ax + ay * ay > sp.range * sp.range || (ax == 0 && ay == 0)) continue;
+          int tx = u.x + ax, ty = u.y + ay;
+          if (!in_bounds(tx, ty)) continue;
+          int g = grid_[cell(tx, ty)];
+          if (g >= 0 && units_[g].owner == enemy) {
+            const Unit& t = units_[g];
+            const int key = (kSpec[t.type].damage > 0 ? 0 : 64) + t.hp;
+            if (key < bkey) { bkey = key; best = (ay + 3) * 7 + (ax + 3); }
+          }
         }
-      }
+    }
     if (best < 0) return false;
     a[0] = A_ATTACK; a[6] = (uint8_t)best;
     return exec(uid, a, rwo);
@@ -390,13 +445,12 @@
   };
   auto chase = [&]() -> bool {
     int e = -1, dist = 1 << 30, b = -1, db = 1 << 30;
-    for (size_t i = 0; i < units_.size(); ++i) {
+    for_owner(enemy, [&](int i) {
       const Unit& t = units_[i];
-      if (!t.alive || t.owner != enemy) continue;
       const int d = std::abs(t.x - u.x) + std::abs(t.y - u.y);
-      if (d < dist) { dist = d; e = (int)i; }
-      if (t.type == BASE && d < db) { db = d; b = (int)i; }
-    }
+      if (d < dist) { dist = d; e = i; }
+      if (t.type == BASE && d < db) { db = d; b = i; }
+    });
     if (e < 0) return false;
     if (kChaseBaseFirst && b >= 0 && db <= dist + kChaseBaseSlack) e = b;
     return move_to(units_[e].x, units_[e].y);
@@ -540,17 +594,13 @@
 
 void MicroRTSSim::bot_act(int player, float* rwo) {
   const int n_workers = cnt_[player][WORKER], n_barracks = cnt_[player][BARRACKS];
-  const int n = (int)units_.size();
+  const int n = n_units_;
   uint16_t cand[32 * 32 + 4], cw[32 * 32 + 4], added[32 * 32 + 4];
-  int nc = 0, w = 0, na = 0;
-  for (int i = 0; i < n; ++i) {
-    const Unit& u = units_[i];
-    const int own = (u.alive != 0) & (u.owner == player);
+  int nc = 0, na = 0;
+  for_idle(player, [&](int i, int widx) {
     cand[nc] = (uint16_t)i;
-    cw[nc] = (uint16_t)w;
-    nc += own & (u.busy == 0);
-    w += own & (u.type == WORKER);
-  }
+    cw[nc++] = (uint16_t)widx;
+  });
   for (int q = 0; q < nc; ++q) {
     const int i = cand[q];
     int widx = cw[q];
@@ -564,7 +614,7 @@
 }
 
 void MicroRTSSim::set_opponent_actions(const uint8_t* a) {
-  std::memcpy(opp_actions_.data(), a, opp_actions_.size());
+  opp_actions_.assign(a, a + (size_t)s_ * s_ * kActComps);
 }
 
 float MicroRTSSim::step(const uint8_t* actions, bool* done, float* raw) {
@@ -572,11 +622,11 @@
   const int nc = s_ * s_;
   uint32_t idle[32 * 32 + 4];
   int n_idle = 0;
-  for (size_t i = 0; i < units_.size(); ++i) {
+  if (validate_) ensure_masks();
+  for_idle(0, [&](int i, int) {
     const Unit& u = units_[i];
-    idle[n_idle] = ((uint32_t)cell(u.x, u.y) << 16) | (uint32_t)i;
-    n_idle += (u.alive != 0) & (u.owner == 0) & (u.busy == 0);
-  }
+    idle[n_idle++] = ((uint32_t)cell(u.x, u.y) << 16) | (uint32_t)i;
+  });
   for (int q = 1; q < n_idle; ++q) {
     const uint32_t key = idle[q];
     int j = q;
@@ -609,19 +659,24 @@
     exec(g, a, rw);
   }
   if (external_opp_) {
-    for (int c = 0; c < nc; ++c) {
-      int rx, ry;
-      map_xy(1, c % s_, c / s_, &rx, &ry);
-      const int g = grid_[cell(rx, ry)];
-      if (g < 0) continue;
-      const Unit& u = units_[g];
-      if (u.owner != 1 || u.busy > 0) continue;
+    uint32_t oidle[32 * 32 + 4];
+    int n_oidle = 0;
+    for_idle(1, [&](int i, int) {
+      const Unit& u = units_[i];
+      oidle[n_oidle++] = ((uint32_t)(nc - 1 - cell(u.x, u.y)) << 16) | (uint32_t)i;
+    });
+    for (int q = 1; q < n_oidle; ++q) {
+      const uint32_t key = oidle[q];
+      int j = q;
+      for (; j > 0 && oidle[j - 1] > key; --j) oidle[j] = oidle[j - 1];
+      oidle[j] = key;
+    }
+    if (!opp16_ && opp_actions_.empty()) opp_actions_.assign((size_t)nc * kActComps, 0);
+    for (int q = 0; q < n_oidle; ++q) {
+      const int c = (int)(oidle[q] >> 16), g = (int)(oidle[q] & 0xFFFFu);
       uint8_t otmp[kActComps];
-      const uint8_t* ap = &opp_actions_[(size_t)c * kActComps];
-      if (opp16_) {
-        mbr::unpack_env_action(opp16_[c], otmp);
-        ap = otmp;
-      }
+      if (opp16_) mbr::unpack_env_action(opp16_[c], otmp);
+      const uint8_t* ap = opp16_ ? otmp : &opp_actions_[(size_t)c * kActComps];
       if (ap[0] >= 6) continue;
       if (validate_ && !getbit(&mask_p1_[(size_t)c * kMaskWords], ap[0])) continue;
       uint8_t a[7];
@@ -649,23 +704,37 @@
     last_winner_ = -1;
   }
   int rows_n = 0, rows_idle = 0;
-  if (!d && rows_out_) {
-    uint32_t spill;
-    for (Unit& u : units_) {
-      const int16_t b = u.busy, nb = (int16_t)(b - (u.alive && b > 0));
-      u.act = (b > 0 && nb == 0 && u.alive) ? (int8_t)A_NOOP : u.act;
-      u.busy = nb;
-      const int live = u.alive != 0;
-      rows_idle += live & (u.owner == 0) & (u.act == A_NOOP);
-      *(rows_n < nc ? rows_out_ + rows_n : &spill) = row_entry(u, 0);
-      rows_n += live;
-    }
-  } else if (!d) {
-    for (Unit& u : units_) {
-      const int16_t b = u.busy, nb = (int16_t)(b - (u.alive && b > 0));
-      u.act = (b > 0 && nb == 0 && u.alive) ? (int8_t)A_NOOP : u.act;
-      u.busy = nb;
-    }
+  if (!d) {
+    uint32_t lines = 0;
+    auto pass = [&](auto with_rows) {
+      uint32_t* const out = rows_out_;
+      const int nw = (n_units_ + 63) >> 6;
+      for (int w = 0; w < nw; ++w) {
+        SlotWord& sw = slots_[w];
+        uint64_t idle0 = 0, idle1 = 0;
+        for (uint64_t m = sw.live[0] | sw.live[1] | sw.live[2]; m; m &= m - 1) {
+          const int bit = __builtin_ctzll(m);
+          Unit& u = units_[(w << 6) + bit];
+          const int16_t b = u.busy, nb = (int16_t)(b - (b > 0));
+          u.act = (b > 0 && nb == 0) ? (int8_t)A_NOOP : u.act;
+          u.busy = nb;
+          idle0 |= (uint64_t)((nb == 0) & (u.owner == 0)) << bit;
+          idle1 |= (uint64_t)((nb == 0) & (u.owner == 1)) << bit;
+          const int c = cell(u.x, u.y);
+          const int lo = std::max(c - s_, 0) >> 5, hi = std::min(c + s_, nc - 1) >> 5;
+          lines |= (((2u << hi) - 1u) & ~((1u << lo) - 1u)) & (0u - (uint32_t)((nb == 0) & (u.owner >= 0)));
+          if (with_rows) {
+            rows_idle += (u.owner == 0) & (u.act == A_NOOP);
+            out[rows_n++] = row_entry(u, 0);
+          }
+        }
+        sw.idle[0] = idle0;
+        sw.idle[1] = idle1;
+      }
+    };
+    if (rows_out_) pass(std::true_type{});
+    else pass(std::false_type{});
+    grid_lines_ = lines;
   }
   float r = 0.f;
   for (int i = 0; i < kNumRewards; ++i) r += rw_[i] * rw[i];
@@ -677,10 +746,7 @@
   }
   rows_n_ = rows_n;
   rows_idle_ = rows_idle;
-  if (!d) {
-    if (validate_) compute_mask(0, mask_);
-    if (external_opp_ && validate_) compute_mask(1, mask_p1_);
-  }
+  mask_stale_ = true;
   return r;
 }
 
@@ -722,27 +788,24 @@
 void MicroRTSSim::write_obs_codes_as(int player, uint16_t* out) const {
   const int nc = s_ * s_;
   std::memset(out, 0, (size_t)nc * sizeof(uint16_t));
-  for (const Unit& u : units_) {
-    if (!u.alive) continue;
+  for_all_live([&](int i) {
+    const Unit& u = units_[i];
     int px, py;
     map_xy(player, u.x, u.y, &px, &py);
     const int own = u.owner < 0 ? 0 : (u.owner == player ? 1 : 2);
     out[cell(px, py)] = mbr::cell_code(std::min<int>(std::max<int>(u.hp, 0), 4),
                                        std::min<int>(std::max<int>(u.res, 0), 4), own, u.type,
                                        u.act);
-  }
+  });
 }
 
 int MicroRTSSim::write_obs_code_list(uint32_t* entries, int* idle_own, int player) const {
-  const int S = s_ * s_;
-  uint32_t spill;
   int n = 0, idle = 0;
-  for (const Unit& u : units_) {
-    const int live = u.alive != 0;
-    idle += live & (u.owner == player) & (u.act == A_NOOP);
-    *(n < S ? entries + n : &spill) = row_entry(u, player);
-    n += live;
-  }
+  for_all_live([&](int i) {
+    const Unit& u = units_[i];
+    idle += (u.owner == player) & (u.act == A_NOOP);
+    entries[n++] = row_entry(u, player);
+  });
   if (idle_own) *idle_own += idle;
   return n;
 }
@@ -778,9 +841,11 @@
 }
 
 void MicroRTSSim::write_mask(uint32_t* out) const {
+  ensure_masks();
   std::memcpy(out, mask_.data(), mask_.size() * sizeof(uint32_t));
 }
 void MicroRTSSim::write_mask_p1(uint32_t* out) const {
+  ensure_masks();
   std::memcpy(out, mask_p1_.data(), mask_p1_.size() * sizeof(uint32_t));
 }
 
@@ -794,6 +859,7 @@
 }
 
 void MicroRTSSim::write_mask_dense(uint8_t* out) const {
+  ensure_masks();
   const int nc = s_ * s_;
   for (int c = 0; c < nc; ++c)
     for (int j = 0; j < kMaskBits; ++j)
diff --git a/microbeast_amd/csrc/env/microrts_sim.h b/microbeast_amd/csrc/env/microrts_sim.h
--- a/microbeast_amd/csrc/env/microrts_sim.h
+++ b/microbeast_amd/csrc/env/microrts_sim.h
@@ -1,4 +1,5 @@
 #pragma once
+#include <cstddef>
 #include <cstdint>
 #include <vector>
 #include <string>
@@ -39,7 +40,14 @@
 class MicroRTSSim {
  public:
   MicroRTSSim(int size, int max_steps, int bot, uint64_t seed,
-              const float* reward_weight );
+              const float* reward_weight , void* state = nullptr);
+  ~MicroRTSSim();
+  MicroRTSSim(const MicroRTSSim&) = delete;
+  MicroRTSSim& operator=(const MicroRTSSim&) = delete;
+  static size_t grid_bytes(int size) { return ((size_t)size * size * sizeof(int16_t) + 63) & ~(size_t)63; }
+  static size_t state_bytes(int size) {
+    return grid_bytes(size) + ((((size_t)size * size + 4) * sizeof(Unit) + 63) & ~(size_t)63);
+  }
   void reset();
   float step(const uint8_t* actions, bool* done, float* raw_rewards );
   void write_obs(uint32_t* out) const;
@@ -47,11 +55,15 @@
   void write_obs_dense(float* out) const;
   void write_mask_dense(uint8_t* out) const;
   int size() const { return s_; }
+  static constexpr size_t kHotBytes = 256;
+  void prefetch_object() const {
+    for (size_t o = 0; o < kHotBytes; o += 64) __builtin_prefetch((const char*)this + o);
+  }
   void prefetch() const {
-    const char* u = (const char*)units_.data();
-    for (size_t o = 0; o < units_.size() * sizeof(Unit); o += 64) __builtin_prefetch(u + o);
-    const char* g = (const char*)grid_.data();
-    for (size_t o = 0; o < grid_.size() * sizeof(int16_t); o += 64) __builtin_prefetch(g + o);
+    const char* u = (const char*)units_;
+    for (size_t o = 0; o < (size_t)n_units_ * sizeof(Unit); o += 64) __builtin_prefetch(u + o);
+    const char* g = (const char*)grid_;
+    for (uint32_t m = grid_lines_; m; m &= m - 1) __builtin_prefetch(g + 64 * __builtin_ctz(m));
   }
   int bot() const { return bot_; }
   void set_bot(int b) { bot_ = b; }
@@ -59,17 +71,14 @@
   int ticks() const { return tick_; }
   void set_external_opponent(bool on) {
     external_opp_ = on;
-    if (on && validate_) compute_mask(1, mask_p1_);
+    mask_stale_ = true;
   }
   void write_obs_p1(uint32_t* out) const;
   void write_mask_p1(uint32_t* out) const;
   void set_opponent_actions(const uint8_t* actions_p1);
   void set_validate(bool on) {
     validate_ = on;
-    if (on) {
-      compute_mask(0, mask_);
-      if (external_opp_) compute_mask(1, mask_p1_);
-    }
+    mask_stale_ = true;
   }
   float step_packed(const uint16_t* env_actions, bool* done);
   float step_packed_list(const uint16_t* env_actions, bool* done, uint32_t* entries, int* n,
@@ -85,7 +94,10 @@
   int count_units(int owner, int type) const {
     if (owner < 0 || owner > 1) {
       int n = 0;
-      for (const Unit& u : units_) n += u.alive && u.owner == owner && (type < 0 || u.type == type);
+      for (int i = 0; i < n_units_; ++i) {
+        const Unit& u = units_[i];
+        n += u.alive && u.owner == owner && (type < 0 || u.type == type);
+      }
       return n;
     }
     if (type >= 0) return cnt_[owner][type];
@@ -103,18 +115,24 @@
   int last_winner_ = -1;
   bool external_opp_ = false;
   bool validate_ = true;
-  std::vector<uint8_t> act_buf_;
-  std::vector<Unit> units_;
-  std::vector<int16_t> grid_;
-  std::vector<uint32_t> mask_;
-  std::vector<uint32_t> mask_p1_;
-  std::vector<uint8_t> opp_actions_;
+  static constexpr int kLiveWords = (32 * 32 + 4 + 63) / 64;
+  int n_units_ = 0;
+  uint32_t grid_lines_ = ~0u;
+  mutable bool mask_stale_ = true;
   int cnt_[2][8] = {};
+  int16_t* grid_ = nullptr;
+  Unit* units_ = nullptr;
   const uint16_t* p16_ = nullptr;
   const uint16_t* opp16_ = nullptr;
   uint32_t* rows_out_ = nullptr;
   int rows_n_ = 0, rows_idle_ = 0;
   int last_add_ = -1;
+  struct SlotWord { uint64_t live[3], idle[2], worker[2]; };
+  SlotWord slots_[kLiveWords] = {};
+  void* own_state_ = nullptr;
+  mutable std::vector<uint32_t> mask_;
+  mutable std::vector<uint32_t> mask_p1_;
+  std::vector<uint8_t> opp_actions_;
 
   uint32_t rand_u32();
   float rand_unit();
@@ -132,11 +150,37 @@
   int add_unit(int type, int owner, int x, int y, int res = 0);
   void kill(int uid);
   void compute_mask(int player, std::vector<uint32_t>& out) const;
+  void ensure_masks() const;
+  template <class F>
+  void for_live(unsigned owners, F f) const {
+    const int nw = (n_units_ + 63) >> 6;
+    const uint64_t k0 = 0ull - (owners & 1u), k1 = 0ull - ((owners >> 1) & 1u),
+                   k2 = 0ull - ((owners >> 2) & 1u);
+    for (int w = 0; w < nw; ++w)
+      for (uint64_t m = (slots_[w].live[0] & k0) | (slots_[w].live[1] & k1) | (slots_[w].live[2] & k2);
+           m; m &= m - 1)
+        f((w << 6) + __builtin_ctzll(m));
+  }
+  template <class F>
+  void for_idle(int player, F f) const {
+    const int nw = (n_units_ + 63) >> 6;
+    int wbase = 0;
+    for (int w = 0; w < nw; ++w) {
+      const uint64_t wk = slots_[w].worker[player];
+      for (uint64_t m = slots_[w].idle[player]; m; m &= m - 1) {
+        const int b = __builtin_ctzll(m);
+        f((w << 6) + b, wbase + __builtin_popcountll(wk & ((1ull << b) - 1)));
+      }
+      wbase += __builtin_popcountll(wk);
+    }
+  }
+  template <class F> void for_owner(int owner, F f) const { for_live(1u << (owner + 1), f); }
+  template <class F> void for_all_live(F f) const { for_live(7u, f); }
   void unit_mask(const Unit& u, int player, uint32_t* w) const;
   bool exec(int uid, const uint8_t* a, float* rw);
   void bot_act(int player, float* rw_opp);
   void bot_unit(int uid, int player, float* rw_opp, int n_workers, int n_barracks, int widx);
-  int nearest(int uid, int owner_filter, int type_filter, int* dist) const;
+  int nearest(int uid, int owner, int type_filter, int* dist) const;
   int dir_toward(const Unit& u, int tx, int ty) const;
   void map_xy(int player, int x, int y, int* ox, int* oy) const;
 };
diff --git a/microbeast_amd/csrc/runtime/engine.cpp b/microbeast_amd/csrc/runtime/engine.cpp
--- a/microbeast_amd/csrc/runtime/engine.cpp
+++ b/microbeast_amd/csrc/runtime/engine.cpp
@@ -315,25 +315,24 @@
       const int g = (wid + k) % NG;
       Group& G = *groups_[g];
       if (G.phase.load(std::memory_order_acquire) != ENV_BUSY) continue;
+      int n_done = 0, n_idle = 0;
+      std::chrono::steady_clock::time_point t0;
       for (;;) {
         int e = G.next_env.fetch_add(chunk_);
         if (e >= E) break;
         int e1 = std::min(e + chunk_, E);
         const int a0 = g * E;
-        auto t0 = std::chrono::steady_clock::now();
+        if (n_done == 0) t0 = std::chrono::steady_clock::now();
         try {
-          if (inject_fault_.exchange(0) != 0)
+          if (inject_fault_.load(std::memory_order_relaxed) != 0 && inject_fault_.exchange(0) != 0)
             throw std::runtime_error("injected env-worker fault (--fault_inject_every)");
           if (sparse_ && G.selfplay)
-            G.idle.fetch_add(env_->step_range_lists_sp(a0 + e, a0 + e1, h_act_list_,
-                                                       h_act_list_p1_, h_code_list_,
-                                                       h_code_list_p1_, list_stride_, h_reward_,
-                                                       h_done_, &log_, G.opp_version),
-                             std::memory_order_relaxed);
+            n_idle += env_->step_range_lists_sp(a0 + e, a0 + e1, h_act_list_, h_act_list_p1_,
+                                                h_code_list_, h_code_list_p1_, list_stride_,
+                                                h_reward_, h_done_, &log_, G.opp_version);
           else if (sparse_)
-            G.idle.fetch_add(env_->step_range_lists(a0 + e, a0 + e1, h_act_list_, h_code_list_,
-                                                    list_stride_, h_reward_, h_done_, &log_),
-                             std::memory_order_relaxed);
+            n_idle += env_->step_range_lists(a0 + e, a0 + e1, h_act_list_, h_code_list_,
+                                             list_stride_, h_reward_, h_done_, &log_);
           else if (G.selfplay)
             env_->step_range_codes_sp(a0 + e, a0 + e1, h_act16_, h_act16_p1_, h_codes_, h_res_,
                                       h_codes_p1_, h_res_p1_, h_reward_, h_done_, &log_,
@@ -345,12 +344,16 @@
           fail("env worker " + std::to_string(wid) + ": " + ex.what());
           return;
         }
+        n_done += e1 - e;
+      }
+      if (n_done) {
+        did = true;
         env_ns_.fetch_add(std::chrono::duration_cast<std::chrono::nanoseconds>(
                               std::chrono::steady_clock::now() - t0).count(),
                           std::memory_order_relaxed);
-        frames_.fetch_add(e1 - e, std::memory_order_relaxed);
-        did = true;
-        if (G.remaining.fetch_sub(e1 - e) == e1 - e) {
+        frames_.fetch_add(n_done, std::memory_order_relaxed);
+        G.idle.fetch_add(n_idle, std::memory_order_relaxed);
+        if (G.remaining.fetch_sub(n_done) == n_done) {
           G.t_ready_ns.store(std::chrono::duration_cast<std::chrono::nanoseconds>(
                                  std::chrono::steady_clock::now().time_since_epoch()).count(),
                              std::memory_order_relaxed);
diff --git a/microbeast_amd/csrc/runtime/vec_env.cpp b/microbeast_amd/csrc/runtime/vec_env.cpp
--- a/microbeast_amd/csrc/runtime/vec_env.cpp
+++ b/microbeast_amd/csrc/runtime/vec_env.cpp
@@ -2,7 +2,10 @@
 
 #include <algorithm>
 #include <atomic>
+#include <cstdlib>
+#include <new>
 #include <random>
+#include <stdexcept>
 #include <thread>
 
 namespace mb {
@@ -10,13 +13,34 @@
 VecEnv::VecEnv(int size, int n_envs, int max_steps, uint64_t seed, const std::vector<int>& bots,
                const float* rw, int env_index_base)
     : size_(size), base_(env_index_base) {
-  for (int i = 0; i < n_envs; ++i) {
-    int bot = bots.empty() ? (int)BOT_COAC : bots[i % bots.size()];
-    sims_.emplace_back(new MicroRTSSim(size, max_steps, bot,
-                                       seed * 1000003ull + (uint64_t)(env_index_base + i), rw));
+  if (size < 1 || size > 32) throw std::invalid_argument("VecEnv: map size must be 1..32");
+  const size_t hdr = (sizeof(MicroRTSSim) + 63) & ~(size_t)63;
+  const size_t stride = hdr + MicroRTSSim::state_bytes(size);
+  if (n_envs > 0) {
+    arena_ = std::aligned_alloc(64, stride * (size_t)n_envs);
+    if (!arena_) throw std::bad_alloc();
+  }
+  sims_.reserve(n_envs > 0 ? n_envs : 0);
+  try {
+    for (int i = 0; i < n_envs; ++i) {
+      int bot = bots.empty() ? (int)BOT_COAC : bots[i % bots.size()];
+      char* p = (char*)arena_ + stride * (size_t)i;
+      sims_.push_back(new (p) MicroRTSSim(size, max_steps, bot,
+                                          seed * 1000003ull + (uint64_t)(env_index_base + i), rw,
+                                          p + hdr));
+    }
+  } catch (...) {
+    for (MicroRTSSim* s : sims_) s->~MicroRTSSim();
+    std::free(arena_);
+    throw;
   }
   ep_ret_.assign(n_envs, 0.f);
   ep_len_.assign(n_envs, 0);
+}
+
+VecEnv::~VecEnv() {
+  for (MicroRTSSim* s : sims_) s->~MicroRTSSim();
+  std::free(arena_);
 }
 
 void VecEnv::reset(uint32_t* obs, uint32_t* mask) {
@@ -148,9 +172,8 @@
                               float* ep_return, int32_t* ep_step) {
   const size_t S = (size_t)size_ * size_;
   for (int i = e0; i < e1; ++i) {
-    if (i + 2 < e1) __builtin_prefetch(sims_[i + 2].get());
+    prefetch_ahead(i, e1);
     if (i + 1 < e1) {
-      sims_[i + 1]->prefetch();
       for (size_t o = 0; o < S * 2; o += 64) {
         __builtin_prefetch((const char*)(actions + (i + 1) * S) + o);
         __builtin_prefetch((char*)(codes + (i + 1) * S) + o, 1);
@@ -189,8 +212,8 @@
                                 EpisodeLog* log, int opponent) {
   const size_t S = (size_t)size_ * size_;
   thread_local std::vector<uint16_t> dense, dense_opp;
-  dense.assign(S, 0);
-  dense_opp.assign(S, 0);
+  if (dense.size() != S) dense.assign(S, 0);
+  if (dense_opp.size() != S) dense_opp.assign(S, 0);
   auto expand = [&](const uint32_t* row, std::vector<uint16_t>& out, uint16_t keep) {
     const uint32_t na = std::min<uint32_t>(row[0] & 0xFFFFu, (uint32_t)S);
     for (uint32_t k = 1; k <= na; ++k) {
@@ -200,7 +223,11 @@
   };
   int idle = 0;
   for (int i = e0; i < e1; ++i) {
-    if (i + 1 < e1) sims_[i + 1]->prefetch();
+    prefetch_ahead(i, e1);
+    if (i + 1 < e1) {
+      __builtin_prefetch(act_lists + (size_t)(i + 1) * stride);
+      __builtin_prefetch(opp_lists + (size_t)(i + 1) * stride);
+    }
     MicroRTSSim& sim = *sims_[i];
     const bool sp = sim.external_opponent();
     const uint32_t* arow = act_lists + (size_t)i * stride;
@@ -239,13 +266,10 @@
   const size_t S = (size_t)size_ * size_;
   int idle = 0;
   thread_local std::vector<uint16_t> dense;
-  dense.assign(S, 0);
-  for (int i = e0; i < e1; ++i) {
-    if (i + 2 < e1) __builtin_prefetch(sims_[i + 2].get());
-    if (i + 1 < e1) {
-      sims_[i + 1]->prefetch();
-      __builtin_prefetch(act_lists + (size_t)(i + 1) * stride);
-    }
+  if (dense.size() != S) dense.assign(S, 0);
+  for (int i = e0; i < e1; ++i) {
+    prefetch_ahead(i, e1);
+    if (i + 1 < e1) __builtin_prefetch(act_lists + (size_t)(i + 1) * stride);
     const uint32_t* arow = act_lists + (size_t)i * stride;
     const uint32_t na = std::min<uint32_t>(arow[0] & 0xFFFFu, (uint32_t)S);
     for (uint32_t k = 1; k <= na; ++k) {
@@ -281,8 +305,7 @@
                                  float* ep_return, int32_t* ep_step) {
   const size_t S = (size_t)size_ * size_;
   for (int i = e0; i < e1; ++i) {
-    if (i + 2 < e1) __builtin_prefetch(sims_[i + 2].get());
-    if (i + 1 < e1) sims_[i + 1]->prefetch();
+    prefetch_ahead(i, e1);
     MicroRTSSim& sim = *sims_[i];
     const bool sp = sim.external_opponent();
     bool d = false;
diff --git a/microbeast_amd/csrc/runtime/vec_env.h b/microbeast_amd/csrc/runtime/vec_env.h
--- a/microbeast_amd/csrc/runtime/vec_env.h
+++ b/microbeast_amd/csrc/runtime/vec_env.h
@@ -40,6 +40,9 @@
  public:
   VecEnv(int size, int n_envs, int max_steps, uint64_t seed, const std::vector<int>& bots,
          const float* reward_weight, int env_index_base = 0);
+  ~VecEnv();
+  VecEnv(const VecEnv&) = delete;
+  VecEnv& operator=(const VecEnv&) = delete;
   int num_envs() const { return (int)sims_.size(); }
   int size() const { return size_; }
   void reset(uint32_t* obs, uint32_t* mask);
@@ -74,7 +77,12 @@
  private:
   int size_;
   int base_;
-  std::vector<std::unique_ptr<MicroRTSSim>> sims_;
+  void* arena_ = nullptr;
+  std::vector<MicroRTSSim*> sims_;
+  void prefetch_ahead(int i, int e1) const {
+    if (i + 2 < e1) sims_[i + 2]->prefetch_object();
+    if (i + 1 < e1) sims_[i + 1]->prefetch();
+  }
   std::vector<float> ep_ret_;
   std::vector<int32_t> ep_len_;
 };
```

Measured after the change: 21.02 million. 2.5% lower.
